# Francis-Rings/MotionEditor

Hardware: AMD Instinct MI355X
Metric: denoise-steps/sec, 24f x 512^2 two-branch UNet3D+ControlNet(+adapter+K/V injection) (higher is better)
Workload: dtype f16

## Files before the change

motioneditor_amd/csrc/gemm.hip:

```cpp
#include "me_common.h"
#include "../../include/motioned.h"
#include <stdio.h>
#include <stdlib.h>

namespace {

constexpr int BK = 64;
#ifndef WIDE_TERMS
#define WIDE_TERMS 0
#endif
constexpr int STAGE_REG = 0, STAGE_GLDS = 1, STAGE_BUF = 2;
constexpr int ROWEPI_FLAG = 1 << 30, TILEORDER_FLAG = 1 << 29;

template <bool NT = false>
__device__ __forceinline__ void st16(f16* p, uint4 v) {
  if constexpr (NT) {
    typedef unsigned u32x4 __attribute__((ext_vector_type(4)));
    __builtin_nontemporal_store((u32x4){v.x, v.y, v.z, v.w}, reinterpret_cast<u32x4*>(p));
  } else {
    *reinterpret_cast<uint4*>(p) = v;
  }
}
template <bool NT = false>
__device__ __forceinline__ void st8(f16* p, uint2 v) {
  if constexpr (NT) {
    typedef unsigned u32x2 __attribute__((ext_vector_type(2)));
    __builtin_nontemporal_store((u32x2){v.x, v.y}, reinterpret_cast<u32x2*>(p));
  } else {
    *reinterpret_cast<uint2*>(p) = v;
  }
}

__device__ uint4 g_zero16;

struct RowInfo {
  int base, y0, x0;
  bool valid;
};

__device__ __forceinline__ RowInfo make_row(const me_gemm_args& a, int m) {
  RowInfo r;
  r.valid = m < a.M;
  r.base = m;
  r.y0 = 0;
  r.x0 = 0;
  if (!r.valid) return r;
  if (a.gather == ME_GATHER_CONV3) {
    const int hw = a.Hout * a.Wout;
    const int img = m / hw;
    const int rem = m - img * hw;
    const int oy = rem / a.Wout;
    const int ox = rem - oy * a.Wout;
    r.base = img * a.Hin * a.Win;
    r.y0 = oy * a.stride - (a.pad0 ? 0 : 1);
    r.x0 = ox * a.stride - (a.pad0 ? 0 : 1);
  } else if (a.gather == ME_GATHER_TCONV) {
    const int bf = m / a.npix;
    r.y0 = bf % a.frames;
    r.x0 = (bf / a.frames) * a.npix + (m - bf * a.npix);
  }
  return r;
}

__device__ __forceinline__ int src_row(const me_gemm_args& a, const RowInfo& r, int tap) {
  if (!r.valid) return -1;
  if (a.gather == ME_GATHER_DENSE) return r.base;
  if (a.gather == ME_GATHER_CONV3) {
    const int ky = tap / 3, kx = tap - ky * 3;
    const int iy = r.y0 + ky, ix = r.x0 + kx;
    const int sh = a.ups ? 1 : 0;
    const int Hv = a.Hin << sh, Wv = a.Win << sh;
    if (iy < 0 || iy >= Hv || ix < 0 || ix >= Wv) return -1;
    if (a.ups == 2 && ((iy | ix) & 1)) return -1;
    return r.base + (iy >> sh) * a.Win + (ix >> sh);
  }
  const int dt = tap - 1;
  const int ftot = a.frames_total > 0 ? a.frames_total : a.frames;
  const int gf = a.frame0 + r.y0, gs = gf + dt;
  if (gs < 0 || gs >= ftot || gs / a.chunk != gf / a.chunk) return -1;
  const int ls = r.y0 + dt;
  if (ls >= 0 && ls < a.frames) return r.base + dt * a.npix;
  const int hb = ls < 0 ? a.halo_prev : a.halo_next;
  return hb < 0 ? -1 : hb + r.x0;
}

template <int NT, int MT, int WN>
__device__ __forceinline__ void init_acc(const me_gemm_args& a, f32x4 (&acc)[NT][MT], int n0, int wn, int lane, bool use_bias = true) {
  const f16* __restrict__ bias = use_bias ? reinterpret_cast<const f16*>(a.bias) : nullptr;
  const int nb = n0 + wn * WN + (lane >> 4) * 4;
  const float inv_alpha = bias ? 1.0f / a.alpha : 0.f;
#pragma unroll
  for (int j = 0; j < NT; ++j) {
    U64 b;
    b.u = (bias && nb + 16 * j < a.N) ? *reinterpret_cast<const uint2*>(bias + nb + 16 * j) : make_uint2(0u, 0u);
    const f32x4 v = {(float)b.e[0] * inv_alpha, (float)b.e[1] * inv_alpha, (float)b.e[2] * inv_alpha, (float)b.e[3] * inv_alpha};
#pragma unroll
    for (int i = 0; i < MT; ++i) acc[j][i] = v;
  }
}

template <int NT, int MT>
__device__ __forceinline__ void ln_fold_acc(const me_gemm_args& a, f32x4 (&acc)[NT][MT], int mbase, int nbase, int lane) {
  const float* __restrict__ st = reinterpret_cast<const float*>(a.ln_stats);
  const float* __restrict__ cs = reinterpret_cast<const float*>(a.ln_colsum);
  const float* __restrict__ cv = reinterpret_cast<const float*>(a.ln_cvec);
  const float invK = 1.0f / (float)a.K;
  float nmean[MT], rstd[MT];
#pragma unroll
  for (int i = 0; i < MT; ++i) {
    const int m = min(mbase + i * 16 + (lane & 15), a.M - 1);
    float s1 = 0.f, s2 = 0.f;
    for (int p = 0; p < a.ln_parts; ++p) {
      const f32x2 v = *reinterpret_cast<const f32x2*>(st + (long)p * a.ln_stride + 2 * (long)m);
      s1 += v[0];
      s2 += v[1];
    }
    const float mu = s1 * invK;
    const float var = __builtin_fmaf(-mu, mu, s2 * invK);
    nmean[i] = -mu;
    rstd[i] = rsqrtf(fmaxf(var, 0.f) + a.ln_eps);
  }
#pragma unroll
  for (int j = 0; j < NT; ++j) {
    const int n = nbase + j * 16 + (lane >> 4) * 4;
    f32x4 s = {0.f, 0.f, 0.f, 0.f}, c = {0.f, 0.f, 0.f, 0.f};
    if (n < a.N) {
      s = *reinterpret_cast<const f32x4*>(cs + n);
      c = *reinterpret_cast<const f32x4*>(cv + n);
    }
#pragma unroll
    for (int i = 0; i < MT; ++i)
#pragma unroll
      for (int r = 0; r < 4; ++r) acc[j][i][r] = __builtin_fmaf(rstd[i], __builtin_fmaf(nmean[i], s[r], acc[j][i][r]), c[r]);
  }
}

constexpr int LN_LDS_BYTES = 12288, LN_LDS_COLSUM = 8192, LN_LDS_CVEC = 10240;
template <int NT, int MT>
__device__ __forceinline__ void ln_fold_acc_lds(const me_gemm_args& a, f32x4 (&acc)[NT][MT], const char* img, int rloc, int cloc, int lane) {
  const float invK = 1.0f / (float)a.K;
  uint2 v[MT][4];
#pragma unroll
  for (int i = 0; i < MT; ++i) {
    const int row = rloc + i * 16 + (lane & 15);
#pragma unroll
    for (int p = 0; p < 4; ++p) v[i][p] = *reinterpret_cast<const uint2*>(img + p * 2048 + row * 8);
  }
  float nmean[MT], rstd[MT];
#pragma unroll
  for (int i = 0; i < MT; ++i) {
    float s1 = 0.f, s2 = 0.f;
#pragma unroll
    for (int p = 0; p < 4; ++p) {
      s1 += __uint_as_float(v[i][p].x);
      s2 += __uint_as_float(v[i][p].y);
    }
    const float mu = s1 * invK;
    const float var = __builtin_fmaf(-mu, mu, s2 * invK);
    nmean[i] = -mu;
    rstd[i] = rsqrtf(fmaxf(var, 0.f) + a.ln_eps);
  }
#pragma unroll
  for (int j = 0; j < NT; ++j) {
    const int col = cloc + j * 16 + (lane >> 4) * 4;
    const uint4 su = *reinterpret_cast<const uint4*>(img + LN_LDS_COLSUM + col * 4), cu = *reinterpret_cast<const uint4*>(img + LN_LDS_CVEC + col * 4);
    const f32x4 s = {__uint_as_float(su.x), __uint_as_float(su.y), __uint_as_float(su.z), __uint_as_float(su.w)};
    const f32x4 c = {__uint_as_float(cu.x), __uint_as_float(cu.y), __uint_as_float(cu.z), __uint_as_float(cu.w)};
#pragma unroll
    for (int i = 0; i < MT; ++i)
#pragma unroll
      for (int r = 0; r < 4; ++r) acc[j][i][r] = __builtin_fmaf(rstd[i], __builtin_fmaf(nmean[i], s[r], acc[j][i][r]), c[r]);
  }
}

template <int F, int NT, int MT, int WN, class RowFn>
__device__ __forceinline__ void epilogue_rows(const me_gemm_args& a, f32x4 (&acc)[NT][MT], RowFn rowfn, int m0, int n0, int wn, int lane, f16* sC, int CLD) {
  static_assert(F >= 0 && (F & 1) == 0, "specialised epilogue");
  const f16* __restrict__ rowvec = reinterpret_cast<const f16*>(a.rowvec);
  const f16* res = reinterpret_cast<const f16*>(a.res);
  const f16* res2 = reinterpret_cast<const f16*>(a.res2);
  f16* C = reinterpret_cast<f16*>(a.C);
  constexpr bool has_rv = (F & 2) != 0, has_res = (F & 4) != 0, has_res2 = (F & 8) != 0;
  const int nb = n0 + wn * WN + (lane >> 4) * 4;
  union P4 { f16x2 h[2]; uint2 u; };
  P4 o[MT][NT];
  int mrow[MT];
  auto rr = [&](int m) { return a.res_rows > 0 ? m % a.res_rows : m; };
  auto rr2 = [&](int m) { return a.res2_rows > 0 ? m % a.res2_rows : m; };
#pragma unroll
  for (int i = 0; i < MT; ++i) {
    mrow[i] = rowfn(i);
#pragma unroll
    for (int j = 0; j < NT; ++j) {
      o[i][j].h[0] = __builtin_convertvector((f32x2){acc[j][i][0] * a.alpha, acc[j][i][1] * a.alpha}, f16x2);
      o[i][j].h[1] = __builtin_convertvector((f32x2){acc[j][i][2] * a.alpha, acc[j][i][3] * a.alpha}, f16x2);
    }
  }
  const bool wide = (F == 0 || WIDE_TERMS) && sC == nullptr && a.N % 8 == 0 && a.ldc % 8 == 0 && (reinterpret_cast<uintptr_t>(a.C) & 15) == 0 &&
                    (!has_rv || (a.ldrv % 8 == 0 && (reinterpret_cast<uintptr_t>(a.rowvec) & 15) == 0)) &&
                    (!has_res || (a.ldr % 8 == 0 && (reinterpret_cast<uintptr_t>(a.res) & 15) == 0)) &&
                    (!has_res2 || (a.ldr2 % 8 == 0 && (reinterpret_cast<uintptr_t>(a.res2) & 15) == 0));
  constexpr int NP = NT / 2;
  const int gq = lane >> 4;
  if (wide) {
    union P8 { f16x2 h[4]; uint4 u; };
    const int nw = n0 + wn * WN + ((gq & 1) ? 16 + 4 * (gq - 1) : 4 * gq);
    P8 w[MT][NP > 0 ? NP : 1];
#pragma unroll
    for (int i = 0; i < MT; ++i)
#pragma unroll
      for (int jp = 0; jp < NP; ++jp) {
        const auto rx = __builtin_amdgcn_permlane16_swap(o[i][2 * jp].u.x, o[i][2 * jp + 1].u.x, false, false);
        const auto ry = __builtin_amdgcn_permlane16_swap(o[i][2 * jp].u.y, o[i][2 * jp + 1].u.y, false, false);
        w[i][jp].u = make_uint4(rx[0], ry[0], rx[1], ry[1]);
      }
    auto add_wide = [&](const f16* src, auto rowoff) {
      P8 t[MT][NP > 0 ? NP : 1];
#pragma unroll
      for (int i = 0; i < MT; ++i) {
        const f16* p = src + rowoff(mrow[i] < 0 ? 0 : mrow[i]) + nw;
#pragma unroll
        for (int jp = 0; jp < NP; ++jp) t[i][jp].u = nw + 32 * jp + 7 < a.N ? *reinterpret_cast<const uint4*>(p + 32 * jp) : make_uint4(0u, 0u, 0u, 0u);
      }
#pragma unroll
      for (int i = 0; i < MT; ++i)
#pragma unroll
        for (int jp = 0; jp < NP; ++jp)
#pragma unroll
          for (int q = 0; q < 4; ++q) w[i][jp].h[q] += t[i][jp].h[q];
    };
    auto add_narrow_last = [&](const f16* src, auto rowoff) {
      if constexpr (NT % 2 == 1) {
#pragma unroll
        for (int i = 0; i < MT; ++i) {
          P4 t;
          t.u = nb + 16 * (NT - 1) < a.N ? *reinterpret_cast<const uint2*>(src + rowoff(mrow[i] < 0 ? 0 : mrow[i]) + nb + 16 * (NT - 1)) : make_uint2(0u, 0u);
          o[i][NT - 1].h[0] += t.h[0];
          o[i][NT - 1].h[1] += t.h[1];
        }
      }
    };
    if constexpr (has_rv) { add_wide(rowvec, [&](int m) { return (long)(m / a.rows_per_vec) * a.ldrv; }); add_narrow_last(rowvec, [&](int m) { return (long)(m / a.rows_per_vec) * a.ldrv; }); }
    if constexpr (has_res) { add_wide(res, [&](int m) { return (long)rr(m) * a.ldr; }); add_narrow_last(res, [&](int m) { return (long)rr(m) * a.ldr; }); }
    if constexpr (has_res2) { add_wide(res2, [&](int m) { return (long)rr2(m) * a.ldr2; }); add_narrow_last(res2, [&](int m) { return (long)rr2(m) * a.ldr2; }); }
    if constexpr (F == 0) {
      if (a.C2) {
        f16* C2 = reinterpret_cast<f16*>(a.C2);
        long hoff[NP + 1];
#pragma unroll
        for (int jp = 0; jp <= NP; ++jp) {
          const int col = jp < NP ? nw + 32 * jp : nb + 16 * (NT - 1);
          const int n2 = col - a.c2_col0, hh = n2 / a.c2_dh;
          hoff[jp] = n2 >= 0 ? (long)hh * a.c2_hs + (n2 - hh * a.c2_dh) : -1;
        }
#pragma unroll
        for (int i = 0; i < MT; ++i) {
          if (mrow[i] < 0) continue;
          f16* crow = C + (long)mrow[i] * a.ldc;
          f16* hrow = C2 + (long)mrow[i] * a.c2_dh;
#pragma unroll
          for (int jp = 0; jp < NP; ++jp)
            if (nw + 32 * jp + 7 < a.N) st16(hoff[jp] >= 0 ? hrow + hoff[jp] : crow + nw + 32 * jp, w[i][jp].u);
          if constexpr (NT % 2 == 1) {
            if (nb + 16 * (NT - 1) < a.N) st8(hoff[NP] >= 0 ? hrow + hoff[NP] : crow + nb + 16 * (NT - 1), o[i][NT - 1].u);
          }
        }
        return;
      }
    }
#pragma unroll
    for (int i = 0; i < MT; ++i) {
      if (mrow[i] < 0) continue;
      f16* crow = C + (long)mrow[i] * a.ldc;
#pragma unroll
      for (int jp = 0; jp < NP; ++jp)
        if (nw + 32 * jp + 7 < a.N) st16(crow + nw + 32 * jp, w[i][jp].u);
      if constexpr (NT % 2 == 1) {
        if (nb + 16 * (NT - 1) < a.N) st8(crow + nb + 16 * (NT - 1), o[i][NT - 1].u);
      }
    }
    return;
  }
  auto add_term = [&](const f16* src, auto rowoff) {
    P4 t[MT][NT];
#pragma unroll
    for (int i = 0; i < MT; ++i) {
      const f16* p = src + rowoff(mrow[i] < 0 ? 0 : mrow[i]) + nb;
#pragma unroll
      for (int j = 0; j < NT; ++j) t[i][j].u = nb + 16 * j < a.N ? *reinterpret_cast<const uint2*>(p + 16 * j) : make_uint2(0u, 0u);
    }
#pragma unroll
    for (int i = 0; i < MT; ++i)
#pragma unroll
      for (int j = 0; j < NT; ++j) {
        o[i][j].h[0] += t[i][j].h[0];
        o[i][j].h[1] += t[i][j].h[1];
      }
  };
  if constexpr (has_rv) add_term(rowvec, [&](int m) { return (long)(m / a.rows_per_vec) * a.ldrv; });
  if constexpr (has_res) add_term(res, [&](int m) { return (long)rr(m) * a.ldr; });
  if constexpr (has_res2) add_term(res2, [&](int m) { return (long)rr2(m) * a.ldr2; });
  if constexpr (F == 0) {
    if (a.C2 && sC == nullptr) {
      f16* C2 = reinterpret_cast<f16*>(a.C2);
#pragma unroll
      for (int j = 0; j < NT; ++j) {
        const int col = nb + 16 * j;
        if (col >= a.N) continue;
        const int n2 = col - a.c2_col0, hh = n2 / a.c2_dh;
        const long hoff = n2 >= 0 ? (long)hh * a.c2_hs + (n2 - hh * a.c2_dh) : -1;
#pragma unroll
        for (int i = 0; i < MT; ++i) {
          if (mrow[i] < 0) continue;
          st8(hoff >= 0 ? C2 + (long)mrow[i] * a.c2_dh + hoff : C + (long)mrow[i] * a.ldc + col, o[i][j].u);
        }
      }
      return;
    }
  }
#pragma unroll
  for (int i = 0; i < MT; ++i) {
    if (mrow[i] < 0) continue;
    f16* crow = C + (long)mrow[i] * a.ldc + nb;
    f16* lrow = sC + (mrow[i] - m0) * CLD + (nb - n0);
#pragma unroll
    for (int j = 0; j < NT; ++j) {
      if (nb + 16 * j >= a.N) continue;
      if (sC) *reinterpret_cast<uint2*>(lrow + 16 * j) = o[i][j].u;
      else st8(crow + 16 * j, o[i][j].u);
    }
  }
}

struct LnOutCtx { int m0, wr, wc, tid; char* red; };
template <int F, int NT, int MT, int WN>
__device__ __forceinline__ void epilogue_rowpass(const me_gemm_args& a, f32x4 (&acc)[NT][MT], int mw0, int nw0, int lane, char* scr, const LnOutCtx& lnx) {
  static_assert(F >= 0 && (F & 1) == 0 && MT % 2 == 0 && WN % 16 == 0, "row-pass epilogue");
  constexpr bool has_rv = (F & 2) != 0, has_res = (F & 4) != 0, has_res2 = (F & 8) != 0;
  constexpr int NCHK = MT / 2, ROWS = 32, CH = WN / 8, PIECES = ROWS * CH, IT = PIECES / 64, PITCH = WN * 2 + 16;
  static_assert(PIECES % 64 == 0, "whole instructions per chunk");
  const f16* __restrict__ rowvec = reinterpret_cast<const f16*>(a.rowvec);
  const f16* res = reinterpret_cast<const f16*>(a.res);
  const f16* res2 = reinterpret_cast<const f16*>(a.res2);
  f16* C = reinterpret_cast<f16*>(a.C);
  union P4 { f16x2 h[2]; uint2 u; };
  union P8 { f16x2 h[4]; uint4 u; };
  P4 o[MT][NT];
#pragma unroll
  for (int i = 0; i < MT; ++i)
#pragma unroll
    for (int j = 0; j < NT; ++j) {
      o[i][j].h[0] = __builtin_convertvector((f32x2){acc[j][i][0] * a.alpha, acc[j][i][1] * a.alpha}, f16x2);
      o[i][j].h[1] = __builtin_convertvector((f32x2){acc[j][i][2] * a.alpha, acc[j][i][3] * a.alpha}, f16x2);
    }
  int prow[IT], pcol[IT], poff[IT];
#pragma unroll
  for (int t = 0; t < IT; ++t) {
    const int p = t * 64 + lane;
    prow[t] = p / CH;
    pcol[t] = nw0 + (p - prow[t] * CH) * 8;
    poff[t] = prow[t] * PITCH + (p - prow[t] * CH) * 16;
  }
  constexpr int TH = MT * 16;
  const int mwc = min(mw0, a.M - 1);
  int v0 = 0, vb = 0x7fffffff, r0 = 0, q0 = 0;
  if constexpr (has_rv) { v0 = mwc / a.rows_per_vec; vb = (v0 + 1) * a.rows_per_vec; }
  if constexpr (has_res) r0 = a.res_rows > 0 ? mwc % a.res_rows : 0;
  if constexpr (has_res2) q0 = a.res2_rows > 0 ? mwc % a.res2_rows : 0;
  auto vrow = [&](int m) { return a.rows_per_vec >= TH ? v0 + (m >= vb ? 1 : 0) : m / a.rows_per_vec; };
  auto wrap = [&](int m, int period, int first) {
    if (period <= 0) return m;
    if (period < TH) return m % period;
    const int x = first + (m - mwc);
    return x >= period ? x - period : x;
  };
  constexpr int NRES = (has_res ? 1 : 0) + (has_res2 ? 1 : 0), NRV = NRES > 0 ? NRES : 1;
  bool rv_once = false;
  P8 rvp[has_rv ? IT : 1];
  if constexpr (has_rv) {
    const int mlast = max(min(mw0 + TH, a.M) - 1, mwc);
    rv_once = vrow(mwc) == vrow(mlast);
    if (rv_once) {
#pragma unroll
      for (int t = 0; t < IT; ++t) rvp[t].u = *reinterpret_cast<const uint4*>(rowvec + (long)vrow(mwc) * a.ldrv + pcol[t]);
    }
  }
  auto load_rv = [&](int c) {
#pragma unroll
    for (int t = 0; t < IT; ++t) {
      const int m = min(mw0 + c * ROWS + prow[t], a.M - 1);
      rvp[t].u = *reinterpret_cast<const uint4*>(rowvec + (long)vrow(m) * a.ldrv + pcol[t]);
    }
  };
  auto load_terms = [&](int c, P8 (&tv)[NRV][IT]) {
#pragma unroll
    for (int t = 0; t < IT; ++t) {
      const int m = min(mw0 + c * ROWS + prow[t], a.M - 1);
      int k = 0;
      if constexpr (has_res) tv[k++][t].u = *reinterpret_cast<const uint4*>(res + (long)wrap(m, a.res_rows, r0) * a.ldr + pcol[t]);
      if constexpr (has_res2) tv[k++][t].u = *reinterpret_cast<const uint4*>(res2 + (long)wrap(m, a.res2_rows, q0) * a.ldr2 + pcol[t]);
    }
  };
  const int wrow = lane & 15, wq = lane >> 4;
  auto park = [&](int c, P8 (&d)[IT]) {
#pragma unroll
    for (int ii = 0; ii < 2; ++ii)
#pragma unroll
      for (int j = 0; j < NT; ++j) *reinterpret_cast<uint2*>(scr + (ii * 16 + wrow) * PITCH + (j * 16 + wq * 4) * 2) = o[c * 2 + ii][j].u;
#pragma unroll
    for (int t = 0; t < IT; ++t) d[t].u = *reinterpret_cast<const uint4*>(scr + poff[t]);
  };
  auto add_rv = [&](P8 (&d)[IT]) {
#pragma unroll
    for (int t = 0; t < IT; ++t)
#pragma unroll
      for (int q = 0; q < 4; ++q) d[t].h[q] += rvp[t].h[q];
  };
  auto add_terms = [&](P8 (&d)[IT], P8 (&tv)[NRV][IT]) {
#pragma unroll
    for (int k = 0; k < NRES; ++k)
#pragma unroll
      for (int t = 0; t < IT; ++t)
#pragma unroll
        for (int q = 0; q < 4; ++q) d[t].h[q] += tv[k][t].h[q];
  };
  long hoff[IT];
  const bool c2 = F == 0 && a.C2 != nullptr;
  if (c2) {
#pragma unroll
    for (int t = 0; t < IT; ++t) {
      const int n2 = pcol[t] - a.c2_col0, hh = n2 / a.c2_dh;
      hoff[t] = n2 >= 0 ? (long)hh * a.c2_hs + (n2 - hh * a.c2_dh) : -1;
    }
  }
  auto store = [&](int c, P8 (&d)[IT]) {
#pragma unroll
    for (int t = 0; t < IT; ++t) {
      const int m = mw0 + c * ROWS + prow[t];
      if (m >= a.M) continue;
      f16* dst = C + (long)m * a.ldc + pcol[t];
      if (c2 && hoff[t] >= 0) dst = reinterpret_cast<f16*>(a.C2) + (long)m * a.c2_dh + hoff[t];
      st16(dst, d[t].u);
    }
  };
  const bool lnout = a.ln_out != nullptr;
  static_assert(CH % 2 == 0, "row sums: half the pieces of a row per half wave");
  f32x2 rsum[NCHK];
  auto row_sums = [&](int c, P8 (&d)[IT]) {
    const f16x2 one2 = {(f16)1.f, (f16)1.f};
#pragma unroll
    for (int t = 0; t < IT; ++t) {
      float s1 = 0.f, s2 = 0.f;
#pragma unroll
      for (int q = 0; q < 4; ++q) {
        s1 = __builtin_amdgcn_fdot2(d[t].h[q], one2, s1, false);
        s2 = __builtin_amdgcn_fdot2(d[t].h[q], d[t].h[q], s2, false);
      }
      const int p = t * 64 + lane;
      *reinterpret_cast<uint2*>(scr + p * 8) = make_uint2(__float_as_uint(s1), __float_as_uint(s2));
    }
    f32x2 acc2 = {0.f, 0.f};
#pragma unroll
    for (int k = 0; k < CH / 2; ++k) {
      const uint2 v = *reinterpret_cast<const uint2*>(scr + ((lane & 31) * CH + (lane >> 5) * (CH / 2) + k) * 8);
      acc2 += f32x2{__uint_as_float(v.x), __uint_as_float(v.y)};
    }
    rsum[c] = f32x2{xor32_sum(acc2[0]), xor32_sum(acc2[1])};
  };
  P8 tv[2][NRV][IT];
  if constexpr (NRES > 0) load_terms(0, tv[0]);
#pragma unroll
  for (int c = 0; c < NCHK; ++c) {
    P8 d[IT];
    if constexpr (has_rv) {
      if (!rv_once) load_rv(c);
    }
    park(c, d);
    if constexpr (has_rv) add_rv(d);
    if constexpr (NRES > 0) {
      add_terms(d, tv[c & 1]);
      if (c + 1 < NCHK) load_terms(c + 1, tv[(c + 1) & 1]);
    }
    store(c, d);
    if (lnout) row_sums(c, d);
  }
  if (lnout) {
    constexpr int GR = MT * 16;
    uint2* red = reinterpret_cast<uint2*>(lnx.red);
    if (lane < 32) {
#pragma unroll
      for (int c = 0; c < NCHK; ++c) red[(lnx.wr * 4 + lnx.wc) * GR + c * 32 + lane] = make_uint2(__float_as_uint(rsum[c][0]), __float_as_uint(rsum[c][1]));
    }
    __syncthreads();
    if (lnx.tid < 2 * GR) {
      const int g = lnx.tid / GR, r = lnx.tid - g * GR, m = lnx.m0 + lnx.tid;
      f32x2 sum = {0.f, 0.f};
#pragma unroll
      for (int w4 = 0; w4 < 4; ++w4) {
        const uint2 v = red[(g * 4 + w4) * GR + r];
        sum += f32x2{__uint_as_float(v.x), __uint_as_float(v.y)};
      }
      if (m < a.M) *reinterpret_cast<f32x2*>(reinterpret_cast<float*>(a.ln_out) + (long)((nw0 - lnx.wc * WN) / 320) * a.ln_out_stride + 2 * (long)m) = sum;
    }
  }
}

template <int NT, int MT, int WN>
__device__ __forceinline__ void epilogue_geglu_rowpass(const me_gemm_args& a, f32x4 (&acc)[NT][MT], int m0, int n0, int wr, int wc, int lane, char* tile) {
  static_assert(NT == 4 && WN == 64, "256-wide GEGLU tile: 4 waves x 32 output columns");
  constexpr int NO = NT / 2, GR = MT * 16;
  f16* C = reinterpret_cast<f16*>(a.C);
  const int wrow = lane & 15, wq = lane >> 4;
#pragma unroll
  for (int i = 0; i < MT; ++i)
#pragma unroll
    for (int jj = 0; jj < NO; ++jj) {
      float v[4];
      {
        const f32x2 v01 = geglu2(f32x2{acc[2 * jj][i][0], acc[2 * jj][i][1]}, f32x2{acc[2 * jj + 1][i][0], acc[2 * jj + 1][i][1]});
        const f32x2 v23 = geglu2(f32x2{acc[2 * jj][i][2], acc[2 * jj][i][3]}, f32x2{acc[2 * jj + 1][i][2], acc[2 * jj + 1][i][3]});
        v[0] = v01[0]; v[1] = v01[1]; v[2] = v23[0]; v[3] = v23[1];
      }
      union { f16x2 h[2]; uint2 u; } o;
      o.h[0] = __builtin_convertvector((f32x2){v[0], v[1]}, f16x2);
      o.h[1] = __builtin_convertvector((f32x2){v[2], v[3]}, f16x2);
      const int row = wr * GR + i * 16 + wrow;
      const int col = wc * 32 + jj * 16 + wq * 4;
      const int pos = (col >> 3) ^ (row & 15);
      *reinterpret_cast<uint2*>(tile + row * 256 + pos * 16 + (col & 4) * 2) = o.u;
    }
  __syncthreads();
  const int wave = wr * 4 + wc;
  constexpr int RW = 2 * GR / 8;
  const int Nout0 = n0 / 2;
#pragma unroll
  for (int t = 0; t < RW / 4; ++t) {
    const int p = t * 64 + lane, row = wave * RW + (p >> 4), pos = p & 15;
    const uint4 v = *reinterpret_cast<const uint4*>(tile + row * 256 + pos * 16);
    const int m = m0 + row, n = Nout0 + ((pos ^ (row & 15)) << 3);
    if (m < a.M) st16<true>(C + (long)m * a.ldc + n, v);
  }
}


template <int NT, int MT, int WN, class RowFn>
__device__ __forceinline__ void epilogue_generic(const me_gemm_args& a, f32x4 (&acc)[NT][MT], RowFn rowfn, int m0, int n0, int wn, int lane, f16* sC, int CLD) {
  const f16* __restrict__ rowvec = reinterpret_cast<const f16*>(a.rowvec);
  const f16* res = reinterpret_cast<const f16*>(a.res);
  const f16* res2 = reinterpret_cast<const f16*>(a.res2);
  f16* C = reinterpret_cast<f16*>(a.C);
  const int nq = (lane >> 4) * 4;
#pragma unroll
  for (int i = 0; i < MT; ++i) {
    const int m = rowfn(i);
    if (m < 0) continue;
    const f16* rv = rowvec ? rowvec + (long)(m / a.rows_per_vec) * a.ldrv : nullptr;
#pragma unroll
    for (int j = 0; j < NT; ++j) {
      const int n = n0 + wn * WN + j * 16 + nq;
      if (n >= a.N) continue;
      float v[4];
#pragma unroll
      for (int r = 0; r < 4; ++r) v[r] = acc[j][i][r] * a.alpha;
      if (rv) {
        U64 b;
        b.u = *reinterpret_cast<const uint2*>(rv + n);
#pragma unroll
        for (int r = 0; r < 4; ++r) v[r] += (float)b.e[r];
      }
      if (a.act == 1) {
#pragma unroll
        for (int r = 0; r < 4; ++r) v[r] = fmaxf(v[r], 0.f);
      } else if (a.act == 2) {
#pragma unroll
        for (int r = 0; r < 4; ++r) v[r] = silu_f(v[r]);
      }
      const int mr = a.res_rows > 0 ? m % a.res_rows : m;
      if (res) {
        U64 b;
        b.u = *reinterpret_cast<const uint2*>(res + (long)mr * a.ldr + n);
#pragma unroll
        for (int r = 0; r < 4; ++r) v[r] += (float)b.e[r];
      }
      if (res2) {
        U64 b;
        b.u = *reinterpret_cast<const uint2*>(res2 + (long)(a.res2_rows > 0 ? m % a.res2_rows : m) * a.ldr2 + n);
#pragma unroll
        for (int r = 0; r < 4; ++r) v[r] += (float)b.e[r];
      }
      U64 o;
#pragma unroll
      for (int r = 0; r < 4; ++r) o.e[r] = (f16)v[r];
      if (sC) *reinterpret_cast<uint2*>(sC + (m - m0) * CLD + (n - n0)) = o.u;
      else *reinterpret_cast<uint2*>(C + (long)m * a.ldc + n) = o.u;
    }
  }
}

template <int NT, int MT, int WN, class RowFn>
__device__ __forceinline__ void epilogue_geglu(const me_gemm_args& a, f32x4 (&acc)[NT][MT], RowFn rowfn, int m0, int n0, int wn, int lane, f16* sC, int CLD) {
  f16* C = reinterpret_cast<f16*>(a.C);
  constexpr int NO = NT / 2;
  const int nb = n0 + wn * WN + (lane >> 4) * 4;
  const int nob = (n0 + wn * WN) / 2 + (lane >> 4) * 4;
  const int Nout = a.N / 2;
  union P4 { f16x2 h[2]; uint2 u; };
  P4 o[MT][NO];
  int mrow[MT];
#pragma unroll
  for (int i = 0; i < MT; ++i) {
    mrow[i] = rowfn(i);
#pragma unroll
    for (int jj = 0; jj < NO; ++jj) {
      float v[4];
      {
        const f32x2 v01 = geglu2(f32x2{acc[2 * jj][i][0], acc[2 * jj][i][1]}, f32x2{acc[2 * jj + 1][i][0], acc[2 * jj + 1][i][1]});
        const f32x2 v23 = geglu2(f32x2{acc[2 * jj][i][2], acc[2 * jj][i][3]}, f32x2{acc[2 * jj + 1][i][2], acc[2 * jj + 1][i][3]});
        v[0] = v01[0]; v[1] = v01[1]; v[2] = v23[0]; v[3] = v23[1];
      }
      o[i][jj].h[0] = __builtin_convertvector((f32x2){v[0], v[1]}, f16x2);
      o[i][jj].h[1] = __builtin_convertvector((f32x2){v[2], v[3]}, f16x2);
    }
  }
  const bool wide = sC == nullptr && Nout % 8 == 0 && a.ldc % 8 == 0 && (reinterpret_cast<uintptr_t>(a.C) & 15) == 0;
  constexpr int NP = NO / 2;
  const int gq = lane >> 4;
  const int nw = (n0 + wn * WN) / 2 + ((gq & 1) ? 16 + 4 * (gq - 1) : 4 * gq);
#pragma unroll
  for (int i = 0; i < MT; ++i) {
    const int m = mrow[i];
    if (wide) {
#pragma unroll
      for (int jp = 0; jp < NP; ++jp) {
        const auto rx = __builtin_amdgcn_permlane16_swap(o[i][2 * jp].u.x, o[i][2 * jp + 1].u.x, false, false);
        const auto ry = __builtin_amdgcn_permlane16_swap(o[i][2 * jp].u.y, o[i][2 * jp + 1].u.y, false, false);
        if (m >= 0 && nw + 32 * jp + 7 < Nout) st16<true>(C + (long)m * a.ldc + nw + 32 * jp, make_uint4(rx[0], ry[0], rx[1], ry[1]));
      }
      if constexpr (NO % 2 == 1) {
        if (m >= 0 && nob + 16 * (NO - 1) < Nout) st8<true>(C + (long)m * a.ldc + nob + 16 * (NO - 1), o[i][NO - 1].u);
      }
      continue;
    }
    if (m < 0) continue;
#pragma unroll
    for (int jj = 0; jj < NO; ++jj) {
      if (nb + 32 * jj >= a.N) continue;
      const int no = nob + 16 * jj;
      if (sC) *reinterpret_cast<uint2*>(sC + (m - m0) * CLD + (no - n0 / 2)) = o[i][jj].u;
      else st8<true>(C + (long)m * a.ldc + no, o[i][jj].u);
    }
  }
}

template <int NT, int MT, int WN, class RowFn>
__device__ __forceinline__ void epilogue(const me_gemm_args& a, f32x4 (&acc)[NT][MT], RowFn rowfn, int m0, int n0, int wn, int lane, f16* sC, int CLD) {
  if (a.geglu) return epilogue_geglu<NT, MT, WN>(a, acc, rowfn, m0, n0, wn, lane, sC, CLD);
  const int f = a.act != 0 ? -1 : ((a.rowvec ? 2 : 0) | (a.res ? 4 : 0) | (a.res2 ? 8 : 0));
  switch (f) {
    case 0: return epilogue_rows<0, NT, MT, WN>(a, acc, rowfn, m0, n0, wn, lane, sC, CLD);
    case 2: return epilogue_rows<2, NT, MT, WN>(a, acc, rowfn, m0, n0, wn, lane, sC, CLD);
    case 4: return epilogue_rows<4, NT, MT, WN>(a, acc, rowfn, m0, n0, wn, lane, sC, CLD);
    case 6: return epilogue_rows<6, NT, MT, WN>(a, acc, rowfn, m0, n0, wn, lane, sC, CLD);
    case 12: return epilogue_rows<12, NT, MT, WN>(a, acc, rowfn, m0, n0, wn, lane, sC, CLD);
    default: return epilogue_generic<NT, MT, WN>(a, acc, rowfn, m0, n0, wn, lane, sC, CLD);
  }
}

template <int BM, int BN, int STAGE, int WM = 64>
__global__ __launch_bounds__(BM / WM * 128, WM == 128 ? 1 : 2) void gemm_kernel(const me_gemm_args a) {
  constexpr int NTHR = BM / WM * 128;
  constexpr int RSTR = NTHR / 8;
  constexpr int WN = BN / 2;
  constexpr int NT = WN / 16;
  constexpr int MT = WM / 16;
  constexpr int XROWS = BM / RSTR;
  constexpr int WROWS = BN / RSTR;
  constexpr int LD = STAGE != STAGE_REG ? BK : BK + 8;

  extern __shared__ __attribute__((aligned(16))) char smem[];
  f16* sX = reinterpret_cast<f16*>(smem);
  f16* sW = sX + 2 * BM * LD;

  const int tid = threadIdx.x;
  const int lane = tid & 63;
  const int wave = __builtin_amdgcn_readfirstlane(tid >> 6);
  const int wm = wave >> 1, wn = wave & 1;

  const int nbn = (a.N + BN - 1) / BN;
  const int nbm = (a.M - a.m_off + BM - 1) / BM;
  const int w = xcd_remap(blockIdx.x, nbm * nbn);
  const int tile_n = w % nbn, tile_m = w / nbn;
  const int m0 = a.m_off + tile_m * BM, n0 = tile_n * BN;

  const f16* __restrict__ X = reinterpret_cast<const f16*>(a.X);
  const f16* __restrict__ W = reinterpret_cast<const f16*>(a.W);

  const int taps = a.gather == ME_GATHER_CONV3 ? 9 : (a.gather == ME_GATHER_TCONV ? 3 : 1);
  const int nkc = (a.K + BK - 1) / BK;
  const bool packk = STAGE == STAGE_GLDS && a.gather == ME_GATHER_CONV3 && a.K < BK && BK % a.K == 0;
  const int nit = packk ? (9 * a.K + BK - 1) / BK : taps * nkc;

  int srow, scol;
  if (STAGE != STAGE_REG) {
    srow = wave * 8 + (lane >> 3);
    scol = ((lane & 7) ^ ((4 * (wave & 1) + (lane >> 4)) & 7)) * 8;
  } else {
    srow = tid >> 3;
    scol = (tid & 7) * 8;
  }

  RowInfo rinfo[XROWS];
#pragma unroll
  for (int i = 0; i < XROWS; ++i) rinfo[i] = make_row(a, m0 + srow + RSTR * i);

  long xoff[XROWS];
  int cur_tap = -1;
  auto set_tap = [&](int tap) {
    if (tap != cur_tap) {
      cur_tap = tap;
#pragma unroll
      for (int i = 0; i < XROWS; ++i) {
        const int s = src_row(a, rinfo[i], tap);
        xoff[i] = s < 0 ? -1L : (long)s * a.ldx;
      }
    }
  };

  const int S = STAGE == STAGE_BUF ? a.splits_ : 0;
  const int it0 = S > 1 ? (int)((long)nit * blockIdx.y / S) : 0;
  const int it1 = S > 1 ? (int)((long)nit * (blockIdx.y + 1) / S) : nit;
  f32x4 acc[NT][MT];
  init_acc<NT, MT, WN>(a, acc, n0, wn, lane, S <= 1);

  const int frow = lane & 15;
  const int fg = lane >> 4;

  auto compute = [&](int buf) {
    const f16* bx = sX + buf * BM * LD;
    const f16* bw = sW + buf * BN * LD;
#pragma unroll
    for (int ks = 0; ks < BK / 32; ++ks) {
      f16x8 fx[MT], fw[NT];
#pragma unroll
      for (int i = 0; i < MT; ++i) {
        const int row = wm * WM + i * 16 + frow;
        const int ch = STAGE != STAGE_REG ? ((ks * 4 + fg) ^ ((row >> 1) & 7)) : (ks * 4 + fg);
        fx[i] = *reinterpret_cast<const f16x8*>(bx + row * LD + ch * 8);
      }
#pragma unroll
      for (int j = 0; j < NT; ++j) {
        const int row = wn * WN + j * 16 + frow;
        const int ch = STAGE != STAGE_REG ? ((ks * 4 + fg) ^ ((row >> 1) & 7)) : (ks * 4 + fg);
        fw[j] = *reinterpret_cast<const f16x8*>(bw + row * LD + ch * 8);
      }
#pragma unroll
      for (int j = 0; j < NT; ++j)
#pragma unroll
        for (int i = 0; i < MT; ++i) acc[j][i] = mfma16(fw[j], fx[i], acc[j][i]);
    }
  };

  if constexpr (STAGE == STAGE_BUF) {
    typedef __attribute__((address_space(3))) void* lptr_t;
    constexpr unsigned OOB = 0x80000000u;
    long brow = m0;
    if (a.gather == ME_GATHER_CONV3) brow = (long)(m0 / (a.Hout * a.Wout)) * a.Hin * a.Win;
    else if (a.gather == ME_GATHER_TCONV) brow = m0 > a.npix ? m0 - a.npix : 0;
    const auto xsrd = __builtin_amdgcn_make_buffer_rsrc(const_cast<f16*>(X + brow * a.ldx), 0, OOB, 0x00020000);
    const int wrows = min(a.N - n0, BN);
    const auto wsrd = __builtin_amdgcn_make_buffer_rsrc(const_cast<f16*>(W + (long)n0 * taps * a.K), 0, (unsigned)((long)wrows * taps * a.K * 2), 0x00020000);
    unsigned xo[XROWS], wo[WROWS];
#pragma unroll
    for (int i = 0; i < WROWS; ++i) wo[i] = (unsigned)(((long)(srow + RSTR * i) * taps * a.K + scol) * 2);
    auto set_tap_off = [&](int tap) {
#pragma unroll
      for (int i = 0; i < XROWS; ++i) {
        const int sr = src_row(a, rinfo[i], tap);
        xo[i] = sr < 0 ? OOB : (unsigned)(((long)(sr - brow) * a.ldx + scol) * 2);
      }
    };
    int tap_l = it0 / nkc, kc_l = it0 - (it0 / nkc) * nkc;
    set_tap_off(tap_l);
    auto gload = [&](int buf) {
      char* dx = reinterpret_cast<char*>(sX + buf * BM * LD) + wave * 1024;
      char* dw = reinterpret_cast<char*>(sW + buf * BN * LD) + wave * 1024;
      const int sx = kc_l * (BK * 2), sw = (tap_l * a.K + kc_l * BK) * 2;
#pragma unroll
      for (int i = 0; i < XROWS; ++i) __builtin_amdgcn_raw_ptr_buffer_load_lds(xsrd, (lptr_t)(dx + i * (RSTR * 128)), 16, (int)xo[i], sx, 0, 0);
#pragma unroll
      for (int i = 0; i < WROWS; ++i) __builtin_amdgcn_raw_ptr_buffer_load_lds(wsrd, (lptr_t)(dw + i * (RSTR * 128)), 16, (int)wo[i], sw, 0, 0);
      if (++kc_l == nkc) {
        kc_l = 0;
        if (++tap_l < taps) set_tap_off(tap_l);
      }
    };
    gload(0);
    __syncthreads();
    for (int it = it0; it < it1; ++it) {
      const int buf = (it - it0) & 1;
      if (it + 1 < it1) gload(buf ^ 1);
      compute(buf);
      __syncthreads();
    }
    if (S > 1) {
      float* wk = reinterpret_cast<float*>(a.work) + (long)blockIdx.y * a.M * a.N;
#pragma unroll
      for (int i = 0; i < MT; ++i) {
        const int m = m0 + wm * WM + i * 16 + (lane & 15);
        if (m >= a.M) continue;
#pragma unroll
        for (int j = 0; j < NT; ++j) {
          const int n = n0 + wn * WN + j * 16 + (lane >> 4) * 4;
          if (n < a.N) *reinterpret_cast<f32x4*>(wk + (long)m * a.N + n) = acc[j][i];
        }
      }
      return;
    }
  } else if constexpr (STAGE == STAGE_GLDS) {
    typedef const __attribute__((address_space(1))) void* gptr_t;
    typedef __attribute__((address_space(3))) void* lptr_t;
    const f16* zsrc = reinterpret_cast<const f16*>(&g_zero16);
    auto gload = [&](int it, int buf) {
      int tap = it / nkc;
      int c = (it - tap * nkc) * BK + scol;
      bool kok = c < a.K;
      long wk = (long)tap * a.K + c;
      if (packk) {
        wk = it * BK + scol;
        tap = (int)wk / a.K;
        c = (int)wk - tap * a.K;
        kok = tap < 9;
        if (!kok) tap = 8;
      }
      set_tap(tap);
      char* dx = reinterpret_cast<char*>(sX + buf * BM * LD) + wave * 1024;
      char* dw = reinterpret_cast<char*>(sW + buf * BN * LD) + wave * 1024;
#pragma unroll
      for (int i = 0; i < XROWS; ++i) {
        const f16* src = (kok && xoff[i] >= 0) ? X + xoff[i] + c : zsrc;
        __builtin_amdgcn_global_load_lds((gptr_t)src, (lptr_t)(dx + i * (RSTR * 128)), 16, 0, 0);
      }
#pragma unroll
      for (int i = 0; i < WROWS; ++i) {
        const int n = n0 + srow + RSTR * i;
        const f16* src = (kok && n < a.N) ? W + (long)n * taps * a.K + wk : zsrc;
        __builtin_amdgcn_global_load_lds((gptr_t)src, (lptr_t)(dw + i * (RSTR * 128)), 16, 0, 0);
      }
    };
    gload(0, 0);
    __syncthreads();
    for (int it = 0; it < nit; ++it) {
      const int buf = it & 1;
      if (it + 1 < nit) gload(it + 1, buf ^ 1);
      compute(buf);
      __syncthreads();
    }
  } else {
    uint4 rx[XROWS], rw[WROWS];
    auto gload = [&](int it) {
      const int tap = it / nkc;
      const int c = (it - tap * nkc) * BK + scol;
      set_tap(tap);
      const bool kok = c < a.K;
#pragma unroll
      for (int i = 0; i < XROWS; ++i) rx[i] = (kok && xoff[i] >= 0) ? ldg128(X + xoff[i] + c) : zero128();
#pragma unroll
      for (int i = 0; i < WROWS; ++i) {
        const int n = n0 + srow + RSTR * i;
        rw[i] = (kok && n < a.N) ? ldg128(W + ((long)n * taps + tap) * a.K + c) : zero128();
      }
    };
    auto sstore = [&](int buf) {
      f16* dx = sX + buf * BM * LD;
      f16* dw = sW + buf * BN * LD;
#pragma unroll
      for (int i = 0; i < XROWS; ++i) *reinterpret_cast<uint4*>(dx + (srow + RSTR * i) * LD + scol) = rx[i];
#pragma unroll
      for (int i = 0; i < WROWS; ++i) *reinterpret_cast<uint4*>(dw + (srow + RSTR * i) * LD + scol) = rw[i];
    };
    gload(0);
    sstore(0);
    __syncthreads();
    for (int it = 0; it < nit; ++it) {
      const int buf = it & 1;
      if (it + 1 < nit) gload(it + 1);
      compute(buf);
      if (it + 1 < nit) sstore(buf ^ 1);
      __syncthreads();
    }
  }

  if (a.ln_stats) ln_fold_acc<NT, MT>(a, acc, m0 + wm * WM, n0 + wn * WN, lane);
  const int ncols = a.geglu ? BN / 2 : BN;
  const int Nout = a.geglu ? a.N / 2 : a.N;
  constexpr bool CFITS = (size_t)BM * (BN + 8) <= (size_t)2 * (BM + BN) * LD;
  const bool wide_store = CFITS && (Nout % 8 == 0) && (a.ldc % 8 == 0) && ((reinterpret_cast<uintptr_t>(a.C) & 15) == 0) && !a.C2;
  auto rowfn = [&](int i) {
    const int m = m0 + wm * WM + i * 16 + (lane & 15);
    return m < a.M ? m : -1;
  };
  if (!wide_store) {
    epilogue<NT, MT, WN>(a, acc, rowfn, m0, n0, wn, lane, nullptr, 0);
    return;
  }
  constexpr int CLD = BN + 8;
  f16* sC = reinterpret_cast<f16*>(smem);
  epilogue<NT, MT, WN>(a, acc, rowfn, m0, n0, wn, lane, sC, CLD);
  __syncthreads();
  f16* C = reinterpret_cast<f16*>(a.C);
  const int vpr = ncols / 8;
  const int nb0 = a.geglu ? n0 / 2 : n0;
  for (int idx = tid; idx < BM * vpr; idx += NTHR) {
    const int row = idx / vpr, c8 = (idx - row * vpr) * 8;
    const int m = m0 + row, n = nb0 + c8;
    if (m < a.M && n < Nout) *reinterpret_cast<uint4*>(C + (long)m * a.ldc + n) = *reinterpret_cast<const uint4*>(sC + row * CLD + c8);
  }
}

constexpr int HALO_W = 18, HALO_ROWS = HALO_W * HALO_W, HALO_INSTR = (HALO_ROWS + 7) / 8;
constexpr int HALO_BYTES = HALO_INSTR * 1024, CONVW_BYTES = 320 * 128;

__global__ __launch_bounds__(512, 2) void conv3_halo_kernel(const me_gemm_args a) {
  constexpr int BN = 320, WN = 160, NT = 10, MT = 4;
  extern __shared__ __attribute__((aligned(16))) char smem[];
  char* sH = smem;
  char* sWt = smem + HALO_BYTES;

  const int tid = threadIdx.x;
  const int lane = tid & 63;
  const int wave = __builtin_amdgcn_readfirstlane(tid >> 6);
  const int wm = wave >> 1, wn = wave & 1;

  const int nbn = a.N / BN;
  const int tx_n = a.Win >> 4, ppi = tx_n * (a.Hin >> 4);
  const int hw = a.Hin * a.Win;
  const int w = xcd_remap(blockIdx.x, (a.M / hw) * ppi * nbn);
  const int tile_n = w % nbn, patch = w / nbn;
  const int img = patch / ppi, pr = patch - img * ppi;
  const int ty = pr / tx_n, tx = pr - ty * tx_n;
  const int y0 = ty * 16, x0 = tx * 16, n0 = tile_n * BN;

  const f16* __restrict__ X = reinterpret_cast<const f16*>(a.X);
  const f16* __restrict__ W = reinterpret_cast<const f16*>(a.W);

  const int srow = wave * 8 + (lane >> 3);
  const int scol = ((lane & 7) ^ ((4 * (wave & 1) + (lane >> 4)) & 7)) * 8;
  typedef __attribute__((address_space(3))) void* lptr_t;
  constexpr unsigned OOB = 0x80000000u;
  const auto xsrd = __builtin_amdgcn_make_buffer_rsrc(const_cast<f16*>(X + (long)img * hw * a.ldx), 0, OOB, 0x00020000);
  const auto wsrd = __builtin_amdgcn_make_buffer_rsrc(const_cast<f16*>(W + (long)n0 * 9 * a.K), 0, (unsigned)((long)BN * 9 * a.K * 2), 0x00020000);
  unsigned hoff[6];
#pragma unroll
  for (int i = 0; i < 6; ++i) {
    const int hr = srow + 64 * i;
    unsigned o = OOB;
    if (hr < HALO_ROWS) {
      const int hy = hr / HALO_W, hx = hr - hy * HALO_W;
      const int iy = y0 - 1 + hy, ix = x0 - 1 + hx;
      if (iy >= 0 && iy < a.Hin && ix >= 0 && ix < a.Win) o = (unsigned)(((long)(iy * a.Win + ix) * a.ldx + scol) * 2);
    }
    hoff[i] = o;
  }
  auto load_halo = [&](int kc) {
#pragma unroll
    for (int i = 0; i < 6; ++i) {
      if (wave + 8 * i < HALO_INSTR)
        __builtin_amdgcn_raw_ptr_buffer_load_lds(xsrd, (lptr_t)(sH + (wave + 8 * i) * 1024), 16, (int)hoff[i], kc * (BK * 2), 0, 0);
    }
  };
  unsigned woff[5];
#pragma unroll
  for (int i = 0; i < 5; ++i) woff[i] = (unsigned)(((long)(srow + 64 * i) * 9 * a.K + scol) * 2);
  auto load_w = [&](int tap, int kc, int buf) {
    char* dw = sWt + buf * CONVW_BYTES + wave * 1024;
    const int so = (tap * a.K + kc * BK) * 2;
#pragma unroll
    for (int i = 0; i < 5; ++i) __builtin_amdgcn_raw_ptr_buffer_load_lds(wsrd, (lptr_t)(dw + i * 8192), 16, (int)woff[i], so, 0, 0);
  };

  f32x4 acc[NT][MT];
  init_acc<NT, MT, WN>(a, acc, n0, wn, lane);

  const int frow = lane & 15, fg = lane >> 4;
  auto compute = [&](int tap, int buf) {
    const int ky = tap / 3, kx = tap - ky * 3;
    const char* bw = sWt + buf * CONVW_BYTES;
    const int hbase = (wm * 4 + ky) * HALO_W + kx + frow;
#pragma unroll
    for (int ks = 0; ks < BK / 32; ++ks) {
      f16x8 fx[MT], fw[NT];
#pragma unroll
      for (int i = 0; i < MT; ++i) {
        const int row = hbase + i * HALO_W;
        fx[i] = *reinterpret_cast<const f16x8*>(sH + row * 128 + (((ks * 4 + fg) ^ ((row >> 1) & 7)) << 4));
      }
#pragma unroll
      for (int j = 0; j < NT; ++j) {
        const int row = wn * WN + j * 16 + frow;
        fw[j] = *reinterpret_cast<const f16x8*>(bw + row * 128 + (((ks * 4 + fg) ^ ((row >> 1) & 7)) << 4));
      }
#pragma unroll
      for (int j = 0; j < NT; ++j)
#pragma unroll
        for (int i = 0; i < MT; ++i) acc[j][i] = mfma16(fw[j], fx[i], acc[j][i]);
    }
  };

  const int nkc = a.K / BK;
  load_halo(0);
  load_w(0, 0, 0);
  __syncthreads();
  int it = 0;
  for (int kc = 0; kc < nkc; ++kc) {
    for (int tap = 0; tap < 9; ++tap, ++it) {
      const int buf = it & 1;
      const bool last_tap = tap == 8;
      if (!last_tap) load_w(tap + 1, kc, buf ^ 1);
      else if (kc + 1 < nkc) load_w(0, kc + 1, buf ^ 1);
      compute(tap, buf);
      if (last_tap && kc + 1 < nkc) {
        __syncthreads();
        load_halo(kc + 1);
      }
      __syncthreads();
    }
  }

  auto rowfn = [&](int i) { return img * hw + (y0 + wm * 4 + i) * a.Win + x0 + (lane & 15); };
  epilogue<NT, MT, WN>(a, acc, rowfn, 0, n0, wn, lane, nullptr, 0);
}

template <int BM, int BN, bool GATHER, int EPI>
__global__ __launch_bounds__(512, 2) void gemm8p_kernel(const me_gemm_args a) {
  constexpr int WN = BN / 4, NT = WN / 16, NT0 = (NT + 1) / 2, NT1 = NT / 2;
  constexpr int GR = BM / 2, HALF = GR / 2, MH = HALF / 16, MT = 2 * MH;
  constexpr int NPA = 2 * HALF / 8;
  constexpr int ABYTES = BM * 128, BUFBYTES = (BM + BN) * 128;
  static_assert(BN % 64 == 0 && NT1 >= 1 && HALF % 16 == 0 && NPA >= 8 && NPA <= 16, "wave tile");
  extern __shared__ __attribute__((aligned(16))) char smem[];

  const int tid = threadIdx.x;
  const int lane = tid & 63;
  const int wave = __builtin_amdgcn_readfirstlane(tid >> 6);
  const int wr = wave >> 2, wc = wave & 3;

  const int nbn = (a.N + BN - 1) / BN;
  const int nbm = (a.M - a.m_off + BM - 1) / BM;
  const int w = xcd_remap(blockIdx.x, nbm * nbn);
  int tile_n, tile_m;
  if (a.splits_ & TILEORDER_FLAG) { tile_m = w % nbm; tile_n = w / nbm; }
  else { tile_n = w % nbn; tile_m = w / nbn; }
  const int m0 = a.m_off + tile_m * BM, n0 = tile_n * BN;

  const f16* __restrict__ X = reinterpret_cast<const f16*>(a.X);
  const f16* __restrict__ W = reinterpret_cast<const f16*>(a.W);
  const int taps = !GATHER ? 1 : (a.gather == ME_GATHER_CONV3 ? 9 : (a.gather == ME_GATHER_TCONV ? 3 : 1));
  const int nkc = a.K / BK;
  const int nit = taps * nkc;

  typedef __attribute__((address_space(3))) void* lptr_t;
  constexpr unsigned OOB = 0x80000000u;
  long brow = m0;
  if (GATHER) {
    if (a.gather == ME_GATHER_CONV3) brow = (long)(m0 / (a.Hout * a.Wout)) * a.Hin * a.Win;
    else if (a.gather == ME_GATHER_TCONV) brow = m0 > a.npix ? m0 - a.npix : 0;
  }
  const auto xsrd = __builtin_amdgcn_make_buffer_rsrc(const_cast<f16*>(X + brow * a.ldx), 0, OOB, 0x00020000);
  const int wrows = min(a.N - n0, BN);
  const auto wsrd = __builtin_amdgcn_make_buffer_rsrc(const_cast<f16*>(W + (long)n0 * taps * a.K), 0, (unsigned)((long)wrows * taps * a.K * 2), 0x00020000);

  const int prow = lane >> 3;
  const int scol = ((lane & 7) ^ ((4 * (wave & 1) + (lane >> 4)) & 7)) * 8;
  int rA[2][2], rB0[NT0], rB1[NT1];
#pragma unroll
  for (int i = 0; i < 2; ++i) {
    const int p = wave + 8 * i;
    rA[0][i] = __builtin_amdgcn_readfirstlane((p / (HALF / 8)) * GR + 8 * (p % (HALF / 8)));
    rA[1][i] = __builtin_amdgcn_readfirstlane((p / (HALF / 8)) * GR + HALF + 8 * (p % (HALF / 8)));
  }
  const bool two_a = __builtin_amdgcn_readfirstlane(wave + 8 < NPA ? 1 : 0) != 0;
#pragma unroll
  for (int i = 0; i < NT0; ++i) {
    const int p = wave + 8 * i;
    rB0[i] = __builtin_amdgcn_readfirstlane((p / (2 * NT0)) * WN + 8 * (p % (2 * NT0)));
  }
#pragma unroll
  for (int i = 0; i < NT1; ++i) {
    const int p = wave + 8 * i;
    rB1[i] = __builtin_amdgcn_readfirstlane((p / (2 * NT1)) * WN + 16 * NT0 + 8 * (p % (2 * NT1)));
  }

  unsigned* tab = reinterpret_cast<unsigned*>(smem + 2 * BUFBYTES);
  unsigned xo[2][2];
  if constexpr (GATHER) {
    const int r = tid & 255;
    const RowInfo ri = make_row(a, r < BM ? m0 + r : a.M);
    for (int tap = tid >> 8; tap < taps; tap += 2) {
      const int sr = src_row(a, ri, tap);
      tab[tap * 256 + r] = sr < 0 ? OOB : (unsigned)((long)(sr - brow) * a.ldx * 2);
    }
    __syncthreads();
  } else {
#pragma unroll
    for (int h = 0; h < 2; ++h)
#pragma unroll
      for (int i = 0; i < 2; ++i) {
        const int m = m0 + rA[h][i] + prow;
        xo[h][i] = (m < a.M && (i == 0 || two_a)) ? (unsigned)(((long)(m - brow) * a.ldx + scol) * 2) : OOB;
      }
  }
  unsigned wo0[NT0], wo1[NT1];
#pragma unroll
  for (int i = 0; i < NT0; ++i) wo0[i] = (unsigned)(((long)(rB0[i] + prow) * taps * a.K + scol) * 2);
#pragma unroll
  for (int i = 0; i < NT1; ++i) wo1[i] = (unsigned)(((long)(rB1[i] + prow) * taps * a.K + scol) * 2);

  struct Cur { int tap, kc, tl; };
  Cur cA0 = {0, 0, 0}, cA1 = {0, 0, 0};
  int tB0 = 0, tB1 = 0;
  auto issueA = [&](Cur& c, int half) {
    char* base = smem + (c.tl & 1) * BUFBYTES;
    const int sx = __builtin_amdgcn_readfirstlane((GATHER ? c.kc : c.tl) * (BK * 2));
    const bool live = c.tl < nit;
    unsigned v[2];
#pragma unroll
    for (int i = 0; i < 2; ++i) {
      if constexpr (GATHER) v[i] = tab[__builtin_amdgcn_readfirstlane(min(c.tap, taps - 1)) * 256 + min(rA[half][i] + prow, 255)] + (unsigned)(scol * 2);
      else v[i] = xo[half][i];
    }
    __builtin_amdgcn_raw_ptr_buffer_load_lds(xsrd, (lptr_t)(base + rA[half][0] * 128), 16, (int)(live ? v[0] : OOB), sx, 0, 0);
    if (BM == 256 || two_a) __builtin_amdgcn_raw_ptr_buffer_load_lds(xsrd, (lptr_t)(base + rA[half][1] * 128), 16, (int)(live ? v[1] : OOB), sx, 0, 0);
    ++c.tl;
    if constexpr (GATHER) {
      if (++c.kc == nkc) { c.kc = 0; ++c.tap; }
    }
  };
  auto issueB0 = [&]() {
    char* base = smem + (tB0 & 1) * BUFBYTES + ABYTES;
    const int sw = __builtin_amdgcn_readfirstlane(tB0 * (BK * 2));
    const bool live = tB0 < nit;
#pragma unroll
    for (int i = 0; i < NT0; ++i)
      __builtin_amdgcn_raw_ptr_buffer_load_lds(wsrd, (lptr_t)(base + rB0[i] * 128), 16, (int)(live ? wo0[i] : OOB), sw, 0, 0);
    ++tB0;
  };
  auto issueB1 = [&]() {
    char* base = smem + (tB1 & 1) * BUFBYTES + ABYTES;
    const int sw = __builtin_amdgcn_readfirstlane(tB1 * (BK * 2));
    const bool live = tB1 < nit;
#pragma unroll
    for (int i = 0; i < NT1; ++i)
      __builtin_amdgcn_raw_ptr_buffer_load_lds(wsrd, (lptr_t)(base + rB1[i] * 128), 16, (int)(live ? wo1[i] : OOB), sw, 0, 0);
    ++tB1;
  };

  f32x4 acc[NT][MT];
  init_acc<NT, MT, WN>(a, acc, n0, wc, lane);

  const int frow = lane & 15, fg = lane >> 4;
  const int c0 = (fg ^ ((frow >> 1) & 7)) << 4;
  const int la0 = (wr * GR + frow) * 128 + c0, la1 = la0 ^ 64;
  const int lb0 = ABYTES + (wc * WN + frow) * 128 + c0, lb1 = lb0 ^ 64;
  f16x8 fa[2][MH], fb[2][NT0];
  auto readA = [&](int buf, int half) {
#pragma unroll
    for (int i = 0; i < MH; ++i) {
      fa[0][i] = *reinterpret_cast<const f16x8*>(smem + buf * BUFBYTES + la0 + (half * MH + i) * 2048);
      fa[1][i] = *reinterpret_cast<const f16x8*>(smem + buf * BUFBYTES + la1 + (half * MH + i) * 2048);
    }
  };
  auto readB = [&](int buf, int j0, int nj) {
#pragma unroll
    for (int j = 0; j < NT0; ++j) {
      if (j < nj) {
        fb[0][j] = *reinterpret_cast<const f16x8*>(smem + buf * BUFBYTES + lb0 + (j0 + j) * 2048);
        fb[1][j] = *reinterpret_cast<const f16x8*>(smem + buf * BUFBYTES + lb1 + (j0 + j) * 2048);
      }
    }
  };
  auto cluster = [&](int half, int j0, int nj) {
    __builtin_amdgcn_s_setprio(1);
#pragma unroll
    for (int ks = 0; ks < 2; ++ks)
#pragma unroll
      for (int j = 0; j < NT0; ++j)
        if (j < nj) {
#pragma unroll
          for (int i = 0; i < MH; ++i) acc[j0 + j][half * MH + i] = mfma16(fb[ks][j], fa[ks][i], acc[j0 + j][half * MH + i]);
        }
    __builtin_amdgcn_s_setprio(0);
  };
#define ME_BAR()                               \
  do {                                         \
    __builtin_amdgcn_sched_barrier(0);         \
    asm volatile("" ::: "memory");             \
    __builtin_amdgcn_s_barrier();              \
    asm volatile("" ::: "memory");             \
    __builtin_amdgcn_sched_barrier(0);         \
  } while (0)
#define ME_LGKM0()                                       \
  do {                                                   \
    asm volatile("s_waitcnt lgkmcnt(0)" ::: "memory");   \
    __builtin_amdgcn_sched_barrier(0);                   \
  } while (0)

  auto wait_young = [&]() {
    static_assert(NT1 == 2, "vmcnt literals below");
    if (BM == 256 || two_a) asm volatile("s_waitcnt vmcnt(4)" ::: "memory");
    else asm volatile("s_waitcnt vmcnt(3)" ::: "memory");
  };
  constexpr bool LN_LDS = EPI == 0 && !GATHER;
  if constexpr (LN_LDS) {
    if (a.ln_stats) {
      constexpr int np = 8;
      for (int q = wave; q < np + 4; q += 8) {
        const char* src;
        unsigned range;
        int dst;
        if (q < np) {
          const bool live = (q >> 1) < a.ln_parts;
          src = reinterpret_cast<const char*>(a.ln_stats) + (live ? ((long)(q >> 1) * a.ln_stride + 2 * (long)m0) * 4 : 0L);
          range = live ? (unsigned)min(a.M - m0, BM) * 8u : 0u;
          dst = (q >> 1) * 2048 + (q & 1) * 1024;
        } else {
          const int k = q - np;
          src = reinterpret_cast<const char*>((k >> 1) ? a.ln_cvec : a.ln_colsum) + (long)n0 * 4;
          range = (unsigned)min(a.N - n0, BN) * 4u;
          dst = ((k >> 1) ? LN_LDS_CVEC : LN_LDS_COLSUM) + (k & 1) * 1024;
        }
        const auto srd = __builtin_amdgcn_make_buffer_rsrc(const_cast<char*>(src), 0, range, 0x00020000);
        __builtin_amdgcn_raw_ptr_buffer_load_lds(srd, (lptr_t)(smem + 2 * BUFBYTES + dst), 16, (q & 1) * 1024 + lane * 16, 0, 0, 0);
      }
    }
  }
  issueA(cA0, 0);
  issueB0();
  issueB1();
  issueA(cA1, 1);
  issueA(cA0, 0);
  issueB1();
  wait_young();
  ME_BAR();
  if (wr == 1) ME_BAR();

  for (int t = 0; t < nit; ++t) {
    const int buf = t & 1;
    readB(buf, 0, NT0);
    readA(buf, 0);
    issueA(cA1, 1);
    ME_BAR();
    ME_LGKM0();
    cluster(0, 0, NT0);
    ME_BAR();
    readB(buf, NT0, NT1);
    issueB0();
    ME_BAR();
    ME_LGKM0();
    cluster(0, NT0, NT1);
    ME_BAR();
    readA(buf, 1);
    issueA(cA0, 0);
    ME_BAR();
    ME_LGKM0();
    cluster(1, NT0, NT1);
    ME_BAR();
    readB(buf, 0, NT0);
    issueB1();
    wait_young();
    ME_BAR();
    ME_LGKM0();
    cluster(1, 0, NT0);
    ME_BAR();
  }
  if (wr == 0) ME_BAR();
  asm volatile("s_waitcnt vmcnt(0)" ::: "memory");
#undef ME_BAR
#undef ME_LGKM0

  if constexpr (EPI <= 0) {
    if (a.ln_stats) {
      if constexpr (LN_LDS) ln_fold_acc_lds<NT, MT>(a, acc, smem + 2 * BUFBYTES, wr * GR, wc * WN, lane);
      else ln_fold_acc<NT, MT>(a, acc, m0 + wr * GR, n0 + wc * WN, lane);
    }
  }

  if constexpr (EPI >= 0 && BN == 256) {
    __builtin_amdgcn_s_barrier();
    return epilogue_geglu_rowpass<NT, MT, WN>(a, acc, m0, n0, wr, wc, lane, smem);
  } else if constexpr (EPI >= 0) {
    __builtin_amdgcn_s_barrier();
    char* scr = smem + wave * (32 * (WN * 2 + 16));
    const int mw0 = m0 + wr * GR, nw0 = n0 + wc * WN;
    const LnOutCtx lnx = {m0, wr, wc, tid, smem + 8 * (32 * (WN * 2 + 16))};
    return epilogue_rowpass<EPI, NT, MT, WN>(a, acc, mw0, nw0, lane, scr, lnx);
  } else {
    auto rowfn = [&](int i) {
      const int m = m0 + wr * GR + i * 16 + (lane & 15);
      return m < a.M ? m : -1;
    };
    epilogue<NT, MT, WN>(a, acc, rowfn, m0, n0, wc, lane, nullptr, 0);
  }
}

__global__ __launch_bounds__(256) void gemm_splitk_reduce_kernel(const me_gemm_args a) {
  const int vpr = a.N / 4;
  const long total = (long)a.M * vpr;
  const float* __restrict__ wk = reinterpret_cast<const float*>(a.work);
  const f16* __restrict__ bias = reinterpret_cast<const f16*>(a.bias);
  const f16* __restrict__ rowvec = reinterpret_cast<const f16*>(a.rowvec);
  const f16* res = reinterpret_cast<const f16*>(a.res);
  const f16* res2 = reinterpret_cast<const f16*>(a.res2);
  f16* C = reinterpret_cast<f16*>(a.C);
  const long plane = (long)a.M * a.N;
  for (long idx = (long)blockIdx.x * 256 + threadIdx.x; idx < total; idx += (long)gridDim.x * 256) {
    const int m = (int)(idx / vpr);
    const int n = (int)(idx - (long)m * vpr) * 4;
    f32x4 v = *reinterpret_cast<const f32x4*>(wk + (long)m * a.N + n);
    for (int s_ = 1; s_ < a.splits_; ++s_) v += *reinterpret_cast<const f32x4*>(wk + s_ * plane + (long)m * a.N + n);
    v *= a.alpha;
    if (bias) {
      U64 b;
      b.u = *reinterpret_cast<const uint2*>(bias + n);
#pragma unroll
      for (int r = 0; r < 4; ++r) v[r] += (float)b.e[r];
    }
    U64 rv, r1, r2, o;
    if (rowvec) rv.u = *reinterpret_cast<const uint2*>(rowvec + (long)(m / a.rows_per_vec) * a.ldrv + n);
    if (res) r1.u = *reinterpret_cast<const uint2*>(res + (long)(a.res_rows > 0 ? m % a.res_rows : m) * a.ldr + n);
    if (res2) r2.u = *reinterpret_cast<const uint2*>(res2 + (long)(a.res2_rows > 0 ? m % a.res2_rows : m) * a.ldr2 + n);
    if (a.act == 0) {
#pragma unroll
      for (int r = 0; r < 4; ++r) {
        f16 h = (f16)v[r];
        if (rowvec) h = h + rv.e[r];
        if (res) h = h + r1.e[r];
        if (res2) h = h + r2.e[r];
        o.e[r] = h;
      }
    } else {
#pragma unroll
      for (int r = 0; r < 4; ++r) {
        float f = v[r];
        if (rowvec) f += (float)rv.e[r];
        f = a.act == 1 ? fmaxf(f, 0.f) : silu_f(f);
        if (res) f += (float)r1.e[r];
        if (res2) f += (float)r2.e[r];
        o.e[r] = (f16)f;
      }
    }
    *reinterpret_cast<uint2*>(C + (long)m * a.ldc + n) = o.u;
  }
}

long split_below() {
  const char* e = getenv("ME_GEMM_SPLITK");
  return e ? atol(e) : 400;
}
int choose_split(const me_gemm_args* a, long blocks, int nit) {
  if (a->geglu || a->K % 64 || a->N < 1280 || blocks >= split_below() || nit < 32 || a->C2 || a->m_off || a->ln_stats) return 1;
  int S = (int)((640 + blocks - 1) / blocks);
  if (S > 4) S = 4;
  if (S > nit / 4) S = nit / 4;
  return S < 2 ? 1 : S;
}

int stage_impl() {
  static int impl = -1;
  if (impl < 0) {
    const char* e = getenv("ME_GEMM_STAGE");
    impl = (e && e[0] == 'r') ? STAGE_REG : STAGE_GLDS;
  }
  return impl;
}

long big_min_blocks() {
  static long v = -1;
  if (v < 0) {
    const char* e = getenv("ME_GEMM_BIG_MIN");
    v = e ? atol(e) : 512;
  }
  return v;
}

long halo_min_blocks() {
  static long v = -1;
  if (v < 0) {
    const char* e = getenv("ME_CONV_HALO_MIN");
    v = e ? atol(e) : 512;
  }
  return v;
}

bool conv_halo() {
  static int on = -1;
  if (on < 0) {
    const char* e = getenv("ME_CONV_HALO");
    on = (e && e[0] == '0') ? 0 : 1;
  }
  return on == 1;
}

bool buf_stage() {
  static int on = -1;
  if (on < 0) {
    const char* e = getenv("ME_GEMM_BUF");
    on = (e && e[0] == '0') ? 0 : 1;
  }
  return on == 1;
}

int use_8p() {
  const char* e = getenv("ME_GEMM_8P");
  return e ? atoi(e) : 2;
}

bool row_epilogue() {
  const char* e = getenv("ME_GEMM_ROWEPI");
  return !(e && e[0] == '0');
}

bool tile_order_exp() {
  static int on = -1;
  if (on < 0) {
    const char* e = getenv("ME_GEMM_TILE_ORDER");
    on = (e && e[0] == '1') ? 1 : 0;
  }
  return on == 1;
}

long min_tiles_192() {
  const char* e = getenv("ME_GEMM_8P_192");
  const long v = e ? atol(e) : 192;
  return v > 0 ? v : (1L << 60);
}

long min_tiles_128() {
  const char* e = getenv("ME_GEMM_8P_128");
  const long v = e ? atol(e) : 192;
  return v > 0 ? v : (1L << 60);
}

long geglu_min_tiles() {
  const char* e = getenv("ME_GEMM_GEGLU_MIN");
  return e ? atol(e) : 240;
}

int min_ktiles_192() {
  const char* e = getenv("ME_GEMM_192_MINK");
  return e ? atoi(e) : 4;
}

long n64_below() {
  const char* e = getenv("ME_GEMM_N64_BELOW");
  return e ? atol(e) : 200;
}

bool tile160() {
  static int on = -1;
  if (on < 0) {
    const char* e = getenv("ME_GEMM_TILE160");
    on = (e && e[0] == '0') ? 0 : 1;
  }
  return on == 1;
}

}

extern "C" void me_set_error(const char* msg);
extern "C" void me_set_kernel(const char* name);
extern "C" const char* me_last_kernel(void);

static thread_local bool g_ln_fused = false;

template <int BM, int BN, int STAGE, int WM = 64>
static int launch_gemm(const me_gemm_args* a, hipStream_t st) {
  const size_t lds = (size_t)2 * (BM + BN) * (STAGE != STAGE_REG ? BK : BK + 8) * sizeof(f16);
  static bool attr_set_dev[64] = {};
  int dev_id = 0;
  (void)hipGetDevice(&dev_id);
  bool& attr_set = attr_set_dev[dev_id & 63];
  if (!attr_set) {
    if (hipFuncSetAttribute(reinterpret_cast<const void*>(&gemm_kernel<BM, BN, STAGE, WM>), hipFuncAttributeMaxDynamicSharedMemorySize, (int)lds) != hipSuccess) {
      me_set_error("me_gemm: hipFuncSetAttribute(MaxDynamicSharedMemorySize) failed");
      return ME_EHIP;
    }
    attr_set = true;
  }
  const int nbm = (a->M - a->m_off + BM - 1) / BM, nbn = (a->N + BN - 1) / BN;
  (void)hipGetLastError();
  me_gemm_args b = *a;
  b.splits_ = 0;
  int S = 1;
  if (STAGE == STAGE_BUF && a->work) {
    const int nit = (a->K / 64) * (a->gather == ME_GATHER_CONV3 ? 9 : (a->gather == ME_GATHER_TCONV ? 3 : 1));
    const int Msel = a->sel_rows > a->M ? a->sel_rows : a->M;
    S = choose_split(a, (long)((Msel + BM - 1) / BM) * nbn, nit);
    if ((int64_t)S * a->M * a->N * 4 > a->work_bytes || a->N % 4 || ((uintptr_t)a->work & 15)) S = 1;
  }
  if (S > 1) {
    b.splits_ = S;
    hipLaunchKernelGGL((gemm_kernel<BM, BN, STAGE, WM>), dim3(nbm * nbn, S), dim3(BM / WM * 128), lds, st, b);
    const long vec = (long)a->M * (a->N / 4);
    hipLaunchKernelGGL(gemm_splitk_reduce_kernel, dim3((unsigned)((vec + 255) / 256 < 4096 ? (vec + 255) / 256 : 4096)), dim3(256), 0, st, b);
  } else {
    hipLaunchKernelGGL((gemm_kernel<BM, BN, STAGE, WM>), dim3(nbm * nbn), dim3(BM / WM * 128), lds, st, b);
  }
  {
    char nm[64];
    snprintf(nm, sizeof(nm), "gemm_kernel<%d,%d%s>%s", BM, BN, STAGE == STAGE_REG ? ",reg" : "", S > 1 ? "+splitk" : "");
    me_set_kernel(nm);
  }
  if (hipGetLastError() != hipSuccess) {
    me_set_error("me_gemm: kernel launch failed");
    return ME_EHIP;
  }
  return ME_OK;
}

template <int BM, int BN, bool GATHER, int EPI>
static int launch_gemm8p_epi(const me_gemm_args& b, hipStream_t st) {
  const int lds = 2 * (BM + BN) * 128 + (GATHER ? 9 * 256 * 4 : (EPI == 0 ? LN_LDS_BYTES : 0));
  static bool attr_set_dev[64] = {};
  int dev_id = 0;
  (void)hipGetDevice(&dev_id);
  bool& attr_set = attr_set_dev[dev_id & 63];
  if (!attr_set) {
    if (hipFuncSetAttribute(reinterpret_cast<const void*>(&gemm8p_kernel<BM, BN, GATHER, EPI>), hipFuncAttributeMaxDynamicSharedMemorySize, lds) != hipSuccess) {
      me_set_error("me_gemm: hipFuncSetAttribute(MaxDynamicSharedMemorySize) failed");
      return ME_EHIP;
    }
    attr_set = true;
  }
  const int nbm = (b.M - b.m_off + BM - 1) / BM, nbn = (b.N + BN - 1) / BN;
  hipLaunchKernelGGL((gemm8p_kernel<BM, BN, GATHER, EPI>), dim3(nbm * nbn), dim3(512), lds, st, b);
  return ME_OK;
}

template <int BM, int BN, bool GATHER>
static int launch_gemm8p(const me_gemm_args* a, hipStream_t st) {
  (void)hipGetLastError();
  me_gemm_args b = *a;
  b.splits_ = 0;
  int epi = -1;
  {
    auto al = [](const void* p, int ld) { return p == nullptr || (ld % 8 == 0 && (reinterpret_cast<uintptr_t>(p) & 15) == 0); };
    const int f = (a->rowvec ? 2 : 0) | (a->res ? 4 : 0) | (a->res2 ? 8 : 0);
    if (BN == 320 && row_epilogue() && !a->geglu && a->act == 0 && a->N % 320 == 0 && (f == 0 || f == 2 || f == 4 || f == 6 || f == 12) && al(a->C, a->ldc) &&
        al(a->rowvec, a->ldrv) && al(a->res, a->ldr) && al(a->res2, a->ldr2) && (!a->C2 || f == 0))
      epi = f;
    if (tile_order_exp()) b.splits_ |= TILEORDER_FLAG;
    if (BN == 256 && BM == 256 && row_epilogue() && a->geglu && a->N % 256 == 0 && al(a->C, a->ldc) && !a->C2) epi = 0;
    if (epi >= 0) b.splits_ |= ROWEPI_FLAG;
    g_ln_fused = BN == 320 && epi >= 0 && a->ln_out != nullptr;
    if (!g_ln_fused) b.ln_out = nullptr;
  }
  int rc;
  if constexpr (BN == 256) {
    rc = epi == 0 ? launch_gemm8p_epi<BM, BN, GATHER, 0>(b, st) : launch_gemm8p_epi<BM, BN, GATHER, -1>(b, st);
  } else {
    switch (epi) {
      case 0: rc = launch_gemm8p_epi<BM, BN, GATHER, 0>(b, st); break;
      case 2: rc = launch_gemm8p_epi<BM, BN, GATHER, 2>(b, st); break;
      case 4: rc = launch_gemm8p_epi<BM, BN, GATHER, 4>(b, st); break;
      case 6: rc = launch_gemm8p_epi<BM, BN, GATHER, 6>(b, st); break;
      case 12: rc = launch_gemm8p_epi<BM, BN, GATHER, 12>(b, st); break;
      default: rc = launch_gemm8p_epi<BM, BN, GATHER, -1>(b, st); break;
    }
  }
  if (rc != ME_OK) return rc;
  {
    char nm[64];
    snprintf(nm, sizeof(nm), "gemm8p_kernel<%d,%d,%s>", BM, BN, GATHER ? "true" : "false");
    me_set_kernel(nm);
  }
  if (hipGetLastError() != hipSuccess) {
    me_set_error("me_gemm: kernel launch failed");
    return ME_EHIP;
  }
  return ME_OK;
}

static int launch_conv_halo(const me_gemm_args* a, hipStream_t st) {
  const int lds = HALO_BYTES + 2 * CONVW_BYTES;
  static bool attr_set_dev[64] = {};
  int dev_id = 0;
  (void)hipGetDevice(&dev_id);
  bool& attr_set = attr_set_dev[dev_id & 63];
  if (!attr_set) {
    if (hipFuncSetAttribute(reinterpret_cast<const void*>(&conv3_halo_kernel), hipFuncAttributeMaxDynamicSharedMemorySize, lds) != hipSuccess) {
      me_set_error("me_gemm: hipFuncSetAttribute(MaxDynamicSharedMemorySize) failed");
      return ME_EHIP;
    }
    attr_set = true;
  }
  const long blocks = (long)(a->M / 256) * (a->N / 320);
  (void)hipGetLastError();
  hipLaunchKernelGGL(conv3_halo_kernel, dim3((unsigned)blocks), dim3(512), lds, st, *a);
  me_set_kernel("conv3_halo_kernel");
  if (hipGetLastError() != hipSuccess) {
    me_set_error("me_gemm: kernel launch failed");
    return ME_EHIP;
  }
  return ME_OK;
}

extern "C" int64_t me_gemm_work_bytes(const me_gemm_args* a) {
  if (!a || a->M <= 0 || a->N <= 0 || a->K <= 0 || a->geglu || a->K % 64 || a->N % 4) return 0;
  const int nit = (a->K / 64) * (a->gather == ME_GATHER_CONV3 ? 9 : (a->gather == ME_GATHER_TCONV ? 3 : 1));
  const long blocks = (long)((a->M + 127) / 128) * ((a->N + 159) / 160);
  const int S = choose_split(a, blocks, nit);
  return S > 1 ? (int64_t)4 * a->M * a->N * 4 : 0;
}

static int gemm_dispatch(const me_gemm_args* a, void* stream);

extern "C" int me_gemm(const me_gemm_args* a, void* stream) {
  if (!a || !a->X || !a->W || !a->C) { me_set_error("me_gemm: null pointer"); return ME_EINVAL; }
  if (a->ln_stats) {
    if (a->gather != ME_GATHER_DENSE || a->bias || a->alpha != 1.0f || a->rowvec || a->res || a->res2 || a->act || !a->ln_colsum || !a->ln_cvec || a->ln_parts < 1 || a->ln_parts > 4 || a->ln_stride < 2 * (int64_t)a->M ||
        (a->ln_stride & 1) || ((uintptr_t)a->ln_stats & 7) || (((uintptr_t)a->ln_colsum | (uintptr_t)a->ln_cvec) & 15) || !(a->ln_eps > 0.f)) {
      me_set_error("me_gemm: a LayerNorm-folded launch is dense, has no bias (it is inside ln_cvec), no rowvec / residual / activation and alpha == 1; ln_colsum / ln_cvec fp32 [N] 16-byte aligned, "
                   "ln_stats 8-byte aligned with 1 <= ln_parts <= 4 parts ln_stride >= 2 M floats apart, ln_eps > 0");
      return ME_EINVAL;
    }
  }
  if (a->ln_out && (a->geglu || a->C2 || a->N % 8 || a->N > 1536 || a->ldc % 8 || ((uintptr_t)a->C & 15) || ((uintptr_t)a->ln_out & 7) || a->ln_out_stride < 2 * (int64_t)a->M || (a->ln_out_stride & 1))) {
    me_set_error("me_gemm: ln_out needs a plain fp16 output of N % 8 == 0, N <= 1536 columns (no GEGLU, no head-major panels), ldc % 8 == 0, and parts >= 2 M floats apart");
    return ME_EINVAL;
  }
  g_ln_fused = false;
  const int rc = gemm_dispatch(a, stream);
  if (rc != ME_OK || !a->ln_out || g_ln_fused) return rc;
  char nm[96];
  snprintf(nm, sizeof(nm), "%s", me_last_kernel());
  const int rc2 = me_ln_stats(reinterpret_cast<const f16*>(a->C) + (long)a->m_off * a->ldc, a->ldc, (int64_t)a->M - a->m_off, a->N,
                              reinterpret_cast<float*>(a->ln_out) + 2 * (long)a->m_off, a->ln_out_stride, stream);
  me_set_kernel(nm);
  return rc2;
}

static int gemm_dispatch(const me_gemm_args* a, void* stream) {
  if (a->M <= 0 || a->N <= 0 || a->K <= 0) { me_set_error("me_gemm: non-positive dimension"); return ME_EINVAL; }
  if (a->K % 8 || a->ldx % 8 || a->ldc % 4 || a->N % 4) { me_set_error("me_gemm: K, ldx must be multiples of 8 and N, ldc of 4"); return ME_EINVAL; }
  if (((uintptr_t)a->X | (uintptr_t)a->W) & 15 || ((uintptr_t)a->C & 7)) { me_set_error("me_gemm: misaligned pointer"); return ME_EINVAL; }
  if (a->gather < 0 || a->gather > 2) { me_set_error("me_gemm: bad gather mode"); return ME_EINVAL; }
  if (a->gather == ME_GATHER_CONV3) {
    if (a->Hin <= 0 || a->Win <= 0 || a->Hout <= 0 || a->Wout <= 0 || (a->stride != 1 && a->stride != 2) || a->ups < 0 || a->ups > 2 ||
        (a->pad0 != 0 && a->pad0 != 1) || a->M % (a->Hout * a->Wout)) { me_set_error("me_gemm: bad conv geometry"); return ME_EINVAL; }
  }
  if (a->gather == ME_GATHER_TCONV) {
    const int ftot = a->frames_total > 0 ? a->frames_total : a->frames;
    if (a->frames <= 0 || a->npix <= 0 || a->chunk <= 0 || ftot % a->chunk || (a->m_off == 0 && a->sel_rows <= a->M && a->M % (a->frames * a->npix)) || a->frame0 < 0 ||
        a->frame0 + a->frames > ftot) { me_set_error("me_gemm: bad tconv geometry"); return ME_EINVAL; }
  }
  if (a->rowvec && (a->rows_per_vec <= 0 || a->ldrv % 4 || ((uintptr_t)a->rowvec & 7))) { me_set_error("me_gemm: bad rowvec"); return ME_EINVAL; }
  if (a->res && (a->ldr % 4 || ((uintptr_t)a->res & 7))) { me_set_error("me_gemm: bad residual"); return ME_EINVAL; }
  if (a->res2 && (a->ldr2 % 4 || ((uintptr_t)a->res2 & 7))) { me_set_error("me_gemm: bad second residual"); return ME_EINVAL; }
  if (a->res_rows < 0 || a->res2_rows < 0) { me_set_error("me_gemm: negative res_rows"); return ME_EINVAL; }
  if (a->act < 0 || a->act > 2) { me_set_error("me_gemm: bad activation"); return ME_EINVAL; }
  if (a->bias && ((uintptr_t)a->bias & 7)) { me_set_error("me_gemm: misaligned bias"); return ME_EINVAL; }
  if (a->geglu && (a->N % 32 || a->rowvec || a->res || a->res2 || a->act || a->alpha != 1.0f)) { me_set_error("me_gemm: geglu needs N % 32 == 0, alpha == 1 and no rowvec/res/act"); return ME_EINVAL; }
  if (a->m_off < 0 || a->m_off >= a->M || (a->m_off > 0 && a->gather == ME_GATHER_CONV3)) { me_set_error("me_gemm: m_off must lie in [0, M) and is for dense / TemporalConv launches"); return ME_EINVAL; }
  if (a->C2 && (a->geglu || a->act || a->rowvec || a->res || a->res2 || a->c2_dh <= 0 || a->c2_dh % 8 || a->c2_col0 < 0 || a->c2_col0 % 16 || a->c2_col0 >= a->N ||
                (a->N - a->c2_col0) % a->c2_dh || a->c2_hs % 8 || a->c2_hs < (int64_t)a->M * a->c2_dh || ((uintptr_t)a->C2 & 15) || a->gather == ME_GATHER_CONV3)) {
    me_set_error("me_gemm: head-major output (C2) needs a term-free epilogue, c2_dh % 8 == 0, c2_col0 % 16 == 0, whole heads, c2_hs % 8 == 0 and >= M * c2_dh, 16-byte alignment");
    return ME_EINVAL;
  }
  hipStream_t st = reinterpret_cast<hipStream_t>(stream);
  const bool wide = a->N % 128 == 0 || a->N % 64 != 0;
  if (stage_impl() == STAGE_GLDS) {
    const int Msel = a->sel_rows > a->M ? a->sel_rows : a->M;
    const long big_blocks = (long)((Msel + 255) / 256) * (a->N / 320);
    if (a->gather == ME_GATHER_CONV3 && a->stride == 1 && a->ups == 0 && !a->pad0 && a->N % 320 == 0 && a->K % 64 == 0 && a->Hin % 16 == 0 &&
        a->Win % 16 == 0 && !a->geglu && big_blocks >= halo_min_blocks() && conv_halo())
      return launch_conv_halo(a, st);
    const bool buf = a->K % 64 == 0 && buf_stage();
    const int nit8 = (a->K / 64) * (a->gather == ME_GATHER_CONV3 ? 9 : (a->gather == ME_GATHER_TCONV ? 3 : 1));
    const bool dense = a->gather == ME_GATHER_DENSE;
    if (a->geglu && dense && buf && use_8p() > 0 && nit8 >= use_8p() && a->N % 256 == 0 && (long)((Msel + 255) / 256) * (a->N / 256) >= geglu_min_tiles())
      return launch_gemm8p<256, 256, false>(a, st);
    if (a->N % 320 == 0 && big_blocks >= big_min_blocks()) {
      if (buf && use_8p() > 0 && nit8 >= use_8p()) {
        if (!a->geglu) return dense ? launch_gemm8p<256, 320, false>(a, st) : launch_gemm8p<256, 320, true>(a, st);
        if (dense && a->N % 256 == 0 && (long)((Msel + 255) / 256) * (a->N / 256) >= big_min_blocks()) return launch_gemm8p<256, 256, false>(a, st);
      }
      return buf ? launch_gemm<256, 320, STAGE_BUF>(a, st) : launch_gemm<256, 320, STAGE_GLDS>(a, st);
    }
    if (a->N % 320 == 0 && !a->geglu && buf && use_8p() > 0 && nit8 >= min_ktiles_192() && nit8 >= use_8p() && (long)((Msel + 191) / 192) * (a->N / 320) >= min_tiles_192())
      return dense ? launch_gemm8p<192, 320, false>(a, st) : launch_gemm8p<192, 320, true>(a, st);
    if (dense && a->N % 320 == 0 && !a->geglu && buf && use_8p() > 0 && nit8 >= min_ktiles_192() && nit8 >= use_8p() && (long)((Msel + 127) / 128) * (a->N / 320) >= min_tiles_128())
      return launch_gemm8p<128, 320, false>(a, st);
    const long blocks160 = (long)((Msel + 127) / 128) * ((a->N + 159) / 160);
    {
      const long blocks128 = (long)((Msel + 127) / 128) * ((a->N + 127) / 128);
      if (a->N % 64 == 0 && blocks128 < n64_below()) return buf ? launch_gemm<128, 64, STAGE_BUF>(a, st) : launch_gemm<128, 64, STAGE_GLDS>(a, st);
    }
    if (a->N % 128 == 0 && blocks160 < 512) return buf ? launch_gemm<128, 128, STAGE_BUF>(a, st) : launch_gemm<128, 128, STAGE_GLDS>(a, st);
    if (!a->geglu && a->N % 160 == 0 && tile160()) return buf ? launch_gemm<128, 160, STAGE_BUF>(a, st) : launch_gemm<128, 160, STAGE_GLDS>(a, st);
    if (wide) return buf ? launch_gemm<128, 128, STAGE_BUF>(a, st) : launch_gemm<128, 128, STAGE_GLDS>(a, st);
    return launch_gemm<128, 64, STAGE_GLDS>(a, st);
  }
  return wide ? launch_gemm<128, 128, STAGE_REG>(a, st) : launch_gemm<128, 64, STAGE_REG>(a, st);
}
```

motioneditor_amd/models/graph.py:

```python
from __future__ import annotations

import contextlib
from dataclasses import dataclass
from typing import Callable, List, Optional, Sequence

import torch

from .. import ops, plan, segments
from ..weights import Packed

HEADS = 8
ADAPTER_CHUNK = 8
HEAD_MAJOR_Q = __import__("os").environ.get("ME_HEAD_MAJOR_Q", "1") != "0"
HEAD_MAJOR_KV = __import__("os").environ.get("ME_HEAD_MAJOR_KV", "1") != "0"
SPLIT_SHARDED_TCONV = __import__("os").environ.get("ME_SPLIT_TCONV", "1") != "0"
INPLACE_SKIPS = __import__("os").environ.get("ME_INPLACE_SKIPS", "1") != "0"
LN_FOLD = __import__("os").environ.get("ME_LN_FOLD", "1") != "0"
COND_EMBED_CACHE = True


@dataclass
class Act:
    t: torch.Tensor
    B: int
    f: int
    h: int
    w: int
    cat: Optional[torch.Tensor] = None

    @property
    def N(self) -> int:
        return self.h * self.w

    @property
    def C(self) -> int:
        return self.t.shape[1]

    def like(self, t: torch.Tensor, h: Optional[int] = None, w: Optional[int] = None) -> "Act":
        return Act(t, self.B, self.f, self.h if h is None else h, self.w if w is None else w)

    def rows_of(self, b: int) -> torch.Tensor:
        n = self.f * self.N
        return self.t[b * n:(b + 1) * n]


@dataclass
class AttnCall:
    q: torch.Tensor
    k: torch.Tensor
    v: torch.Tensor
    B: int
    f: int
    N: int
    dh: int
    nk: int
    is_cross: bool
    shard: object = None
    q_items: int = 0

    def run(self, seg_item: torch.Tensor, seg_mode: torch.Tensor, mask: Optional[torch.Tensor] = None) -> torch.Tensor:
        return ops.attention(self.q, self.k, self.v, heads=HEADS, dh=self.dh, n_items=self.B * self.f, nq=self.N, nk=self.nk,
                             seg_item=seg_item, seg_mode=seg_mode, mask=mask, **({"q_items": self.q_items} if self.q_items else {}))


@dataclass
class TemporalCall:
    q: torch.Tensor
    k: torch.Tensor
    v: torch.Tensor
    B: int
    f: int
    N: int
    dh: int
    shard: object = None
    parts: int = 0

    def run(self, kv_map: Optional[Sequence[int]] = None) -> torch.Tensor:
        if self.parts > 1:
            return ops.temporal_attention(self.q, self.k, self.v, heads=HEADS, dh=self.dh, batch=self.B, frames=self.f, npix=self.N, kv_map=kv_map,
                                          kv_parts=self.parts, q_parts=self.parts)
        if self.shard is None:
            return ops.temporal_attention(self.q, self.k, self.v, heads=HEADS, dh=self.dh, batch=self.B, frames=self.f, npix=self.N, kv_map=kv_map)
        sh = self.shard
        return ops.temporal_attention(self.q, self.k, self.v, heads=HEADS, dh=self.dh, batch=self.B, frames=sh.f_total, npix=self.N, kv_map=kv_map,
                                      q_frames=sh.f_loc, q_frame0=sh.frame0, kv_parts=sh.world)


def conv3x3(P: Packed, name: str, x: Act, stride: int = 1, ups: int = 0, **epi) -> Act:
    hv, wv = x.h << ups, x.w << ups
    ho, wo = (hv - 1) // stride + 1, (wv - 1) // stride + 1
    out = ops.gemm(x.t, P.mat(name + ".weight"), M=x.B * x.f * ho * wo, bias=P.vec(name + ".bias"),
                   conv=(x.h, x.w, ho, wo, stride, ups), **epi)
    return x.like(out, ho, wo)


def resnet_block(P: Packed, p: str, x: Act, temb: torch.Tensor, temb_off: int, *, per_frame_stats: bool, eps: float = 1e-5, shard=None,
                 out: Optional[torch.Tensor] = None) -> Act:
    rpg = x.N if per_frame_stats else x.f * x.N
    cout = P.vec(p + ".conv1.bias").shape[0]
    tv = temb[:, temb_off:temb_off + cout]
    rows_per_vec = x.t.shape[0] if temb.shape[0] == 1 else x.f * x.N
    has_t1 = P.has(p + ".temp_conv1.weight") and not P.is_zero(p + ".temp_conv1.weight", p + ".temp_conv1.bias")
    has_t2 = P.has(p + ".temp_conv2.weight") and not P.is_zero(p + ".temp_conv2.weight", p + ".temp_conv2.bias")

    gn = {}
    if shard is not None and not per_frame_stats:
        gn = dict(reduce=shard.allreduce_, rows_per_group_total=shard.f_total * x.N)
    ftot = shard.f_total if shard is not None else x.f
    rows = x.B * x.f * x.N
    h = ops.groupnorm(x.t, P.vec(p + ".norm1.weight"), P.vec(p + ".norm1.bias"), rows_per_group=rpg, eps=eps, silu=True, **gn)
    if has_t1:
        hx = torch.empty((_ext_rows(x, shard), cout), dtype=P.dtype, device=x.t.device)
        h = conv3x3(P, p + ".conv1", x.like(h), out=hx).t
        h = _tconv(P, p + ".temp_conv1", hx, x, ftot, shard, rowvec=tv, rows_per_vec=rows_per_vec, res=h)
    else:
        h = conv3x3(P, p + ".conv1", x.like(h), rowvec=tv, rows_per_vec=rows_per_vec).t
    h = ops.groupnorm(h, P.vec(p + ".norm2.weight"), P.vec(p + ".norm2.bias"), rows_per_group=rpg, eps=eps, silu=True, **gn)
    if P.has(p + ".conv_shortcut.weight"):
        sc = ops.gemm(x.t, P.mat(p + ".conv_shortcut.weight"), bias=P.vec(p + ".conv_shortcut.bias"))
    else:
        sc = x.t
    if has_t2:
        hx = torch.empty((_ext_rows(x, shard), cout), dtype=P.dtype, device=x.t.device)
        h = conv3x3(P, p + ".conv2", x.like(h), out=hx).t
        h = _tconv(P, p + ".temp_conv2", hx, x, ftot, shard, res=h, res2=sc, **({} if out is None else {"out": out}))
    else:
        h = conv3x3(P, p + ".conv2", x.like(h), res=sc, **({} if out is None else {"out": out})).t
    return x.like(h)


def _fold() -> bool:
    return LN_FOLD and not getattr(ops, "recording", False) and getattr(ops, "LN_FOLD", False)


def _gemm_st(*args, **kw):
    if _fold():
        return ops.gemm(*args, ln_out=True, **kw)
    return ops.gemm(*args, **kw), None


class LN:

    def __init__(self, P: Packed, norm: str, x: torch.Tensor, stats: Optional[torch.Tensor] = None):
        self.P, self.norm, self.x, self.stats, self._rows = P, norm, x, stats, None

    def rows(self) -> torch.Tensor:
        if self._rows is None:
            self._rows = ops.layernorm(self.x, self.P.vec(self.norm + ".weight"), self.P.vec(self.norm + ".bias"))
        return self._rows

    def gemm(self, names: Sequence[str], *, geglu_bias: Optional[str] = None, **kw):
        names = list(names)
        geglu = geglu_bias is not None
        if _fold() and self._rows is None:
            if self.stats is None:
                self.stats = ops.ln_stats(self.x)
            w, cs, cv = self.P.ln_fold(self.norm, names, geglu=geglu, bias=geglu_bias)
            return ops.gemm(self.x, w, ln=(self.stats, cs, cv, 1e-5), geglu=geglu, **kw)
        if geglu:
            return ops.gemm(self.rows(), self.P.geglu_mat(names[0]), bias=self.P.geglu_vec(geglu_bias), geglu=True, **kw)
        return ops.gemm(self.rows(), self.P.fused(names) if len(names) > 1 else self.P.mat(names[0]), **kw)


def feed_forward(P: Packed, p: str, n: "LN", res: torch.Tensor, want_stats: bool = False):
    g = n.gemm([p + ".net.0.proj.weight"], geglu_bias=p + ".net.0.proj.bias")
    return (_gemm_st if want_stats else (lambda *a, **k: (ops.gemm(*a, **k), None)))(g, P.mat(p + ".net.2.weight"), bias=P.vec(p + ".net.2.bias"), res=res)


def _ln(P: Packed, p: str, x: torch.Tensor) -> torch.Tensor:
    return ops.layernorm(x, P.vec(p + ".weight"), P.vec(p + ".bias"))


def _qkv(P: Packed, p: str, n: "LN", C: int, shard, B: int = 0, N: int = 0, head_major: bool = False):
    names = [p + ".to_q.weight", p + ".to_k.weight", p + ".to_v.weight"]
    if shard is None:
        if head_major and HEAD_MAJOR_KV and not getattr(ops, "recording", False) and getattr(ops, "HEAD_MAJOR_KV", False):
            if HEAD_MAJOR_Q:
                _, qkv = n.gemm(names, head_major=(0, C // HEADS))
                return qkv[:HEADS], qkv[HEADS:2 * HEADS], qkv[2 * HEADS:]
            q, kv = n.gemm(names, head_major=(C, C // HEADS))
            return q, kv[:HEADS], kv[HEADS:]
        qkv = n.gemm(names)
        return qkv[:, :C], qkv[:, C:2 * C], qkv[:, 2 * C:]
    ext, loc = shard.kv_buffer(n.x.shape[0], 2 * C, B, N, n.x)
    n.gemm(names[1:], out=loc)
    pending = shard.start_kv(ext, B, N, ops.copy_rows)
    q = n.gemm(names[:1])
    kv = shard.finish_kv(pending)
    return q, kv[:, :C], kv[:, C:]


def _temporal_attn(P: Packed, p: str, n: "LN", C: int, B: int, f: int, N: int, dh: int, shard, editor=None, place: str = "") -> torch.Tensor:
    def go(tc):
        return editor(call=tc, is_cross=False, place_in_unet=place, num_heads=HEADS) if editor is not None else tc.run()
    if shard is not None and shard.pixel_sharded(N):
        r = shard.to_pixel_shards(n.rows(), B * f, N, ops.copy_blocks)
        qkv = ops.gemm(r, P.fused([p + ".to_q.weight", p + ".to_k.weight", p + ".to_v.weight"]))
        a = go(TemporalCall(qkv[:, :C], qkv[:, C:2 * C], qkv[:, 2 * C:], B, shard.f_total, N // shard.world, dh, None, shard.world))
        return shard.to_frame_shards(a, B * f, N, ops.copy_blocks)
    q, k, v = _qkv(P, p, n, C, shard)
    return go(TemporalCall(q, k, v, B, f, N, dh, shard))


def _tconv(P: Packed, name: str, h_ext: torch.Tensor, x: "Act", chunk: int, shard, **epi) -> torch.Tensor:
    rows = x.B * x.f * x.N
    if shard is None:
        return ops.gemm(h_ext, P.mat(name + ".weight"), M=rows, bias=P.vec(name + ".bias"), tconv=(x.f, x.N, chunk), **epi)
    if SPLIT_SHARDED_TCONV and x.f >= 3 and getattr(ops, "ROW_RANGE", False) and not ops.gemm_splits_k(rows, P.mat(name + ".weight").shape[0], h_ext.shape[1], 3):
        w, b = P.mat(name + ".weight"), P.vec(name + ".bias")
        out = epi.pop("out", None)
        if out is None:
            out = torch.empty((rows, w.shape[0]), dtype=h_ext.dtype, device=h_ext.device)
        handle = shard.exchange_halos(h_ext, x.B, x.N, ops.copy_rows, defer=True)
        interior = (x.f, x.N, chunk, shard.frame0, shard.f_total, -1, -1)
        for bi in range(x.B):
            ops.gemm(h_ext, w, M=rows, bias=b, tconv=interior, out=out, row_range=((bi * x.f + 1) * x.N, (bi * x.f + x.f - 1) * x.N), **epi)
        hp, hn = shard.finish_halos(handle)
        full = (x.f, x.N, chunk, shard.frame0, shard.f_total, hp, hn)
        bounds = [(0, x.N)] + [((bi * x.f - 1) * x.N, (bi * x.f + 1) * x.N) for bi in range(1, x.B)] + [(rows - x.N, rows)]
        for lo, hi in bounds:
            ops.gemm(h_ext, w, M=rows, bias=b, tconv=full, out=out, row_range=(lo, hi), **epi)
        return out
    hp, hn = shard.exchange_halos(h_ext, x.B, x.N, ops.copy_rows)
    return ops.gemm(h_ext, P.mat(name + ".weight"), M=rows, bias=P.vec(name + ".bias"),
                    tconv=(x.f, x.N, chunk, shard.frame0, shard.f_total, hp, hn), **epi)


def _ext_rows(x: "Act", shard) -> int:
    return x.B * x.f * x.N + (2 * x.B * x.N if shard is not None else 0)


def basic_block(P: Packed, p: str, x: Act, text: Optional[torch.Tensor], text_seg, *, spatial, temporal, place: str,
                sc_attn: bool, has_temp: bool, shard=None, text_kv: Optional[torch.Tensor] = None, expand: int = 1, stats: Optional[torch.Tensor] = None) -> Act:
    t, C = x.t, x.C
    dh = C // HEADS
    sh1 = shard.prev_frame_view() if (shard is not None and sc_attn) else None
    q, k, v = _qkv(P, p + ".attn1", LN(P, p + ".norm1", t, stats), C, sh1, x.B, x.N, head_major=True)
    call = AttnCall(q, k, v, x.B, x.f, x.N, dh, x.N, False, sh1)
    if spatial is not None:
        a = spatial(call=call, is_cross=False, place_in_unet=place, num_heads=HEADS)
    elif sc_attn:
        a = call.run(*segments.prev_cur(x.B, x.f, t.device, sh1))
    else:
        a = call.run(*segments.self_items(x.B * x.f, t.device))
    t, st = _gemm_st(a, P.mat(p + ".attn1.to_out.0.weight"), bias=P.vec(p + ".attn1.to_out.0.bias"), res=t)
    if expand > 1 and text is None:
        raise ValueError("basic_block: expand needs the text cross-attention (that is where the batch entries start to differ)")
    if text is not None:
        q = LN(P, p + ".norm2", t, st).gemm([p + ".attn2.to_q.weight"])
        kv = text_kv if text_kv is not None else ops.gemm(text, P.fused([p + ".attn2.to_k.weight", p + ".attn2.to_v.weight"]))
        call = AttnCall(q, kv[:, :C], kv[:, C:], x.B * expand, x.f, x.N, dh, 77, True, None, x.B * x.f if expand > 1 else 0)
        if spatial is not None:
            a = spatial(call=call, is_cross=True, place_in_unet=place, num_heads=HEADS, text_seg=text_seg)
        else:
            a = call.run(*text_seg)
        if expand > 1:
            ops.SELECT_ROWS_SCALE = 1
        t, st = _gemm_st(a, P.mat(p + ".attn2.to_out.0.weight"), bias=P.vec(p + ".attn2.to_out.0.bias"), res=t, **({"res_rows": t.shape[0]} if expand > 1 else {}))
        if expand > 1:
            x = Act(t, x.B * expand, x.f, x.h, x.w)
    t, st = feed_forward(P, p + ".ff", LN(P, p + ".norm3", t, st), t, want_stats=has_temp)
    if has_temp:
        a = _temporal_attn(P, p + ".attn_temp", LN(P, p + ".norm_temp", t, st), C, x.B, x.f, x.N, dh, shard, temporal, place)
        t = ops.gemm(a, P.mat(p + ".attn_temp.to_out.0.weight"), bias=P.vec(p + ".attn_temp.to_out.0.bias"), res=t)
    return x.like(t)


def transformer2d(P: Packed, p: str, x: Act, text, text_seg, *, spatial=None, temporal=None, place: str = "", sc_attn: bool = True,
                  has_temp: bool = True, shard=None, out: Optional[torch.Tensor] = None, text_kv: Optional[dict] = None, expand: int = 1) -> Act:
    n = ops.groupnorm(x.t, P.vec(p + ".norm.weight"), P.vec(p + ".norm.bias"), rows_per_group=x.N, eps=1e-6, silu=False)
    t, st = _gemm_st(n, P.mat(p + ".proj_in.weight"), bias=P.vec(p + ".proj_in.bias"))
    t = basic_block(P, p + ".transformer_blocks.0", x.like(t), text, text_seg, spatial=spatial, temporal=temporal, place=place,
                    sc_attn=sc_attn, has_temp=has_temp, shard=shard, text_kv=None if text_kv is None else text_kv[p], expand=expand, stats=st).t
    y = ops.gemm(t, P.mat(p + ".proj_out.weight"), bias=P.vec(p + ".proj_out.bias"), res=x.t, **({} if out is None else {"out": out}),
                 **({"res_rows": x.t.shape[0]} if expand > 1 else {}))
    return Act(y, x.B * expand, x.f, x.h, x.w)


def resnet_names(n_up: bool) -> List[str]:
    names = [f"down_blocks.{i}.resnets.{j}" for i in range(4) for j in range(2)] + ["mid_block.resnets.0", "mid_block.resnets.1"]
    if n_up:
        names += [f"up_blocks.{i}.resnets.{j}" for i in range(4) for j in range(3)]
    return names


def time_embedding(P: Packed, t: float, names: List[str], device):
    e = ops.timestep_embed(1, 320, t, device)
    e = ops.gemm(e, P.mat("time_embedding.linear_1.weight"), bias=P.vec("time_embedding.linear_1.bias"), act=2)
    e = ops.gemm(e, P.mat("time_embedding.linear_2.weight"), bias=P.vec("time_embedding.linear_2.bias"), act=2)
    w = P.fused([n + ".time_emb_proj.weight" for n in names])
    b = P.fused_vec([n + ".time_emb_proj.bias" for n in names])
    temb = ops.gemm(e, w, bias=b)
    offs, o = {}, 0
    for n in names:
        offs[n] = o
        o += P.vec(n + ".conv1.bias").shape[0]
    return temb, offs


def attention_block_names(n_up: bool) -> List[str]:
    names = [f"down_blocks.{i}.attentions.{j}" for i in range(3) for j in range(2)] + ["mid_block.attentions.0"]
    if n_up:
        names += [f"up_blocks.{i}.attentions.{j}" for i in range(1, 4) for j in range(3)]
    return names


def text_kv_all(P: Packed, text: torch.Tensor, names: List[str]) -> dict:
    ws = []
    for n in names:
        t = n + ".transformer_blocks.0.attn2."
        ws += [t + "to_k.weight", t + "to_v.weight"]
    kv = ops.gemm(text, P.fused(ws))
    out, o = {}, 0
    for n in names:
        c2 = 2 * P.vec(n + ".norm.weight").shape[0]
        out[n] = kv[:, o:o + c2]
        o += c2
    return out


def adapter_block(P: Packed, p: str, x: Act, src, nb: Optional[int] = None, shard=None) -> torch.Tensor:
    t, C, dev = x.t, x.C, x.t.device
    dh = C // HEADS
    nb = x.B if nb is None else nb
    share = nb != x.B
    if share:
        assert x.B == 1
    rows_x = t.shape[0]
    if shard is None:
        tx = t
    else:
        tx = torch.empty((_ext_rows(x, shard), C), dtype=P.dtype, device=dev)
        ops.copy_rows(tx[:t.shape[0]], t)
    hc = _tconv(P, p + ".block1", tx, x, ADAPTER_CHUNK, shard, act=1)
    hc = ops.gemm(hc, P.mat(p + ".block2.weight"), bias=P.vec(p + ".block2.bias"), res=t)
    sh2 = shard.chunk_view(ADAPTER_CHUNK) if (shard is not None and shard.adapter == "halo") else shard
    q_, k_, v_ = _qkv(P, p + ".attn_temp", LN(P, p + ".norm_temp", t), C, sh2, x.B, x.N)
    a = AttnCall(q_, k_, v_, x.B, x.f, x.N, dh, x.N, False, sh2).run(*segments.first_prev_chunked(x.B, x.f, ADAPTER_CHUNK, dev, sh2))
    a = ops.gemm(a, P.mat(p + ".attn_temp.to_out.0.weight"), bias=P.vec(p + ".attn_temp.to_out.0.bias"), res=t)
    a = _ln(P, p + ".cross_pose_norm", a)
    q = ops.gemm(a, P.mat(p + ".attn_pose.to_q.weight"))
    wkv = P.fused([p + ".attn_pose.to_k.weight", p + ".attn_pose.to_v.weight"])
    if isinstance(src, (list, tuple)):
        n1 = src[0].shape[0]
        kv = torch.empty((len(src) * n1, 2 * C), dtype=P.dtype, device=dev)
        for k, part in enumerate(src):
            ops.gemm(part, wkv, out=kv[k * n1:(k + 1) * n1])
    else:
        kv = ops.gemm(src, wkv)
    seg = segments.self_items(nb * x.f, dev)
    ap = ops.attention(q, kv[:, :C], kv[:, C:], heads=HEADS, dh=dh, n_items=nb * x.f, nq=x.N, nk=x.N, seg_item=seg[0], seg_mode=seg[1],
                       **({"q_items": x.B * x.f} if share else {}))
    a, st = _gemm_st(ap, P.mat(p + ".attn_pose.to_out.0.weight"), bias=P.vec(p + ".attn_pose.to_out.0.bias"), res=a, **({"res_rows": rows_x} if share else {}))
    a, st = feed_forward(P, p + ".ff", LN(P, p + ".ff_norm", a, st), a, want_stats=True)
    at = _temporal_attn(P, p + ".attn_self_temp", LN(P, p + ".norm_self_temp", a, st), C, nb, x.f, x.N, dh, shard)
    return ops.gemm(at, P.mat(p + ".attn_self_temp.to_out.0.weight"), bias=P.vec(p + ".attn_self_temp.to_out.0.bias"), res=a, res2=hc,
                    **({"res2_rows": rows_x} if share else {}))


def adapter_pack(P: Packed, prefix: str = "controlnet_adapter.") -> List[str]:
    for i in range(12):
        p = f"{prefix}body.{i}"
        P.mat(p + ".block1.weight"), P.vec(p + ".block1.bias"), P.mat(p + ".block2.weight"), P.vec(p + ".block2.bias")
        for a in ("attn_temp", "attn_self_temp"):
            P.fused([f"{p}.{a}.to_q.weight", f"{p}.{a}.to_k.weight", f"{p}.{a}.to_v.weight"])
        P.mat(p + ".attn_pose.to_q.weight")
        P.fused([p + ".attn_pose.to_k.weight", p + ".attn_pose.to_v.weight"])
        for a in ("attn_temp", "attn_pose", "attn_self_temp"):
            P.mat(f"{p}.{a}.to_out.0.weight"), P.vec(f"{p}.{a}.to_out.0.bias")
        for n in ("norm_temp", "cross_pose_norm", "ff_norm", "norm_self_temp"):
            P.vec(f"{p}.{n}.weight"), P.vec(f"{p}.{n}.bias")
        P.geglu_mat(p + ".ff.net.0.proj.weight"), P.geglu_vec(p + ".ff.net.0.proj.bias"), P.mat(p + ".ff.net.2.weight"), P.vec(p + ".ff.net.2.bias")
    return sorted(P.trainable_ids(prefix).values())


def unet_tune_pack(P: Packed, names: Sequence[str]) -> List[str]:
    blocks = {f"{b}.transformer_blocks.0": b for b in attention_block_names(True)}
    text_kv = [f"{b}.transformer_blocks.0.attn2.{w}.weight" for b in attention_block_names(True) for w in ("to_k", "to_v")]
    keys, bad = [], []
    for n in names:
        parts = n.split(".")
        head = ".".join(parts[:5]) if parts[0] == "mid_block" else ".".join(parts[:6])
        tail = n[len(head) + 1:]
        if head not in blocks:
            bad.append(n)
            continue
        if tail in ("attn1.to_q.weight", "attn1.to_k.weight", "attn1.to_v.weight", "attn_temp.to_q.weight", "attn_temp.to_k.weight", "attn_temp.to_v.weight"):
            a = tail.split(".")[0]
            P.fused([f"{head}.{a}.to_q.weight", f"{head}.{a}.to_k.weight", f"{head}.{a}.to_v.weight"])
            keys.append("fused:" + "|".join(f"{head}.{a}.to_{x}.weight" for x in "qkv"))
        elif tail == "attn2.to_q.weight" or tail.endswith(("to_out.0.weight", "ff.net.2.weight")) and tail.split(".")[0] in ("attn1", "attn2", "attn_temp", "ff"):
            P.mat(n)
            keys.append("mat:" + n)
        elif tail.endswith(("to_out.0.bias", "ff.net.2.bias")) and tail.split(".")[0] in ("attn1", "attn2", "attn_temp", "ff"):
            P.vec(n)
            keys.append("vec:" + n)
# ... 265 lines not shown
```

motioneditor_amd/ops.py:

```python
from __future__ import annotations

import ctypes as C
from typing import Optional, Sequence, Tuple

import os

import torch

from . import capi
from .capi import AttnArgs, AttnBwdArgs, ConvSmallArgs, GemmArgs, GemmDwArgs, GroupNormArgs, LayerNormArgs, TAttnArgs

F16 = torch.float16


_raw_stream = getattr(torch._C, "_cuda_getCurrentRawStream", None)
_cur_device = getattr(torch._C, "_cuda_getDevice", None)


def _stream() -> int:
    if _raw_stream is not None and _cur_device is not None:
        return _raw_stream(_cur_device())
    return torch.cuda.current_stream().cuda_stream


def _p(t: Optional[torch.Tensor]) -> Optional[int]:
    return None if t is None else t.data_ptr()


def _chk2d(t: torch.Tensor, name: str) -> None:
    if t.dtype != F16 or t.dim() != 2 or t.stride(1) != 1 or not t.is_cuda:
        raise ValueError(f"{name}: expected a CUDA fp16 2-D tensor with unit column stride, got {t.dtype} {tuple(t.shape)} {t.stride()}")


SELECT_ROWS_SCALE = 1
PROFILE = None


def _pb():
    if PROFILE is None:
        return None
    e = torch.cuda.Event(enable_timing=True)
    e.record()
    return e


def _pe(e0, family: str, flops: float, nbytes: float, detail: str = "", kernel: str = "", exec_flops=None) -> None:
    if e0 is None:
        return
    e1 = torch.cuda.Event(enable_timing=True)
    e1.record()
    PROFILE.append((family, flops, nbytes, e0, e1, detail, kernel or family, flops if exec_flops is None else exec_flops))


def _last_kernel() -> str:
    return capi.lib().me_last_kernel().decode()


def empty(rows: int, cols: int, like: torch.Tensor) -> torch.Tensor:
    return torch.empty((rows, cols), dtype=F16, device=like.device)


ATTN_ITEM_ORDER = os.environ.get("ME_ATTN_ITEM_ORDER", "1") != "0"
ROW_RANGE = True
LN_FOLD = True
HEAD_MAJOR_KV = True


def gemm(x: torch.Tensor, w: torch.Tensor, *, M: Optional[int] = None, out: Optional[torch.Tensor] = None,
         bias: Optional[torch.Tensor] = None, rowvec: Optional[torch.Tensor] = None, rows_per_vec: int = 0,
         res: Optional[torch.Tensor] = None, res2: Optional[torch.Tensor] = None, geglu: bool = False, act: int = 0, alpha: float = 1.0,
         conv: Optional[Tuple[int, int, int, int, int, int]] = None,
         tconv: Optional[Tuple[int, ...]] = None, res_rows: int = 0, res2_rows: int = 0, head_major: Optional[Tuple[int, int]] = None,
         row_range: Optional[Tuple[int, int]] = None, ln: Optional[Tuple[torch.Tensor, torch.Tensor, torch.Tensor, float]] = None, ln_out: bool = False):
    _chk2d(x, "gemm.x")
    if w.dtype != F16 or not w.is_contiguous() or w.dim() != 3:
        raise ValueError("gemm.w: expected contiguous fp16 [N, taps, K]")
    N, taps, K = w.shape
    a = GemmArgs()
    a.gather = capi.GATHER_DENSE
    if conv is not None:
        a.gather = capi.GATHER_CONV3
        a.Hin, a.Win, a.Hout, a.Wout, a.stride, a.ups = conv[:6]
        a.pad0 = conv[6] if len(conv) > 6 else 0
        if taps != 9:
            raise ValueError("gemm: conv needs 9 taps")
    elif tconv is not None:
        a.gather = capi.GATHER_TCONV
        a.frames, a.npix, a.chunk = tconv[:3]
        if len(tconv) > 3:
            a.frame0, a.frames_total, a.halo_prev, a.halo_next = tconv[3:]
        if taps != 3:
            raise ValueError("gemm: tconv needs 3 taps")
    elif taps != 1:
        raise ValueError("gemm: dense needs 1 tap")
    if M is None:
        M = x.shape[0]
    if x.shape[1] < K:
        raise ValueError(f"gemm: x has {x.shape[1]} columns < K={K}")
    n_out = N // 2 if geglu else N
    panels = None
    if head_major is not None:
        col0, hdh = head_major
        if out is not None or geglu or (N - col0) % hdh or col0 < 0:
            raise ValueError("gemm: head_major needs whole heads behind col0 >= 0 and allocates its own outputs")
        panels = torch.empty(((N - col0) // hdh, M, hdh), dtype=F16, device=x.device)
        a.C2, a.c2_col0, a.c2_dh, a.c2_hs = panels.data_ptr(), col0, hdh, M * hdh
        n_out = col0
        if col0 == 0:
            out = panels.view(-1)[:8 * M].view(M, 8)
    if out is None:
        if row_range is not None:
            raise ValueError("gemm: row_range writes into a caller-provided `out` of all M rows")
        out = empty(M, n_out, x)
    _chk2d(out, "gemm.out")
    if out.shape[0] < M or out.shape[1] < n_out:
        raise ValueError("gemm: out too small")
    a.X, a.W, a.C = x.data_ptr(), w.data_ptr(), out.data_ptr()
    a.M, a.N, a.K = M, N, K
    if row_range is not None:
        lo, hi = row_range
        if not (0 <= lo < hi <= M) or conv is not None:
            raise ValueError("gemm: row_range must lie inside [0, M) (dense / TemporalConv launches)")
        a.m_off, a.M = lo, hi
        a.sel_rows = max(a.sel_rows, M)
    a.ldx, a.ldc = x.stride(0), out.stride(0)
    a.bias = _p(bias)
    if rowvec is not None:
        _chk2d(rowvec, "gemm.rowvec")
        a.rowvec, a.ldrv, a.rows_per_vec = rowvec.data_ptr(), rowvec.stride(0), rows_per_vec
    if res is not None:
        _chk2d(res, "gemm.res")
        a.res, a.ldr = res.data_ptr(), res.stride(0)
    if res2 is not None:
        _chk2d(res2, "gemm.res2")
        a.res2, a.ldr2 = res2.data_ptr(), res2.stride(0)
    a.geglu = 1 if geglu else 0
    a.act = act
    a.alpha = alpha
    a.res_rows, a.res2_rows = res_rows, res2_rows
    if ln is not None:
        st_, cs_, cv_, eps_ = ln
        if st_.dtype != torch.float32 or st_.dim() != 3 or st_.shape[2] != 2 or st_.stride(2) != 1 or st_.stride(1) != 2 or st_.shape[1] < M \
                or cs_.dtype != torch.float32 or cv_.dtype != torch.float32 or cs_.numel() != N or cv_.numel() != N or not cs_.is_contiguous() or not cv_.is_contiguous():
            raise ValueError("gemm: ln = (fp32 stats [parts, rows, 2], fp32 colsum [N], fp32 cvec [N], eps)")
        a.ln_stats, a.ln_colsum, a.ln_cvec, a.ln_eps = st_.data_ptr(), cs_.data_ptr(), cv_.data_ptr(), eps_
        a.ln_parts, a.ln_stride = st_.shape[0], st_.stride(0)
    so = None
    if ln_out:
        if panels is not None or geglu:
            raise ValueError("gemm: ln_out is for plain row outputs")
        so = torch.empty((n_out // 320 if n_out % 320 == 0 else 1, M, 2), dtype=torch.float32, device=x.device)
        a.ln_out, a.ln_out_stride = so.data_ptr(), so.stride(0)
    if SELECT_ROWS_SCALE > 1:
        a.sel_rows = M * SELECT_ROWS_SCALE
    for r_, n_ in ((res, res_rows), (res2, res2_rows)):
        if r_ is not None and r_.shape[0] < (n_ or M):
            raise ValueError("gemm: residual has fewer rows than the output reads")
    if N >= 1280 and M <= 8192:
        nb = capi.lib().me_gemm_work_bytes(C.byref(a))
        if nb > 0:
            a.work, a.work_bytes = _work(nb, x.device, "splitk").data_ptr(), nb
    e0 = _pb()
    capi.check(capi.lib().me_gemm(C.byref(a), _stream()), "me_gemm")
    if e0 is not None:
        rows_in = (M // (conv[2] * conv[3])) * conv[0] * conv[1] if conv is not None else M
        n_terms = (res is not None) + (res2 is not None)
        n_hm = panels.numel() // M if panels is not None else 0
        _pe(e0, "gemm", 2.0 * M * N * K * taps, 2.0 * (rows_in * K + N * K * taps + M * n_out * (1 + n_terms) + M * n_hm), f"M{M} N{N} K{K} taps{taps}{' geglu' if geglu else ''}{' +b' if bias is not None else ''}{' +rv' if rowvec is not None else ''}"
            f"{' +res' if res is not None else ''}{' +res2' if res2 is not None else ''}{' act' + str(act) if act else ''}{' a' + str(alpha) if alpha != 1.0 else ''}{' ln' if ln is not None else ''}{' lnout' if ln_out else ''}", _last_kernel())
    if panels is not None and n_out == 0:
        return None, panels
    out = out[:M, :n_out] if (out.shape[0] != M or out.shape[1] != n_out) else out
    if so is not None:
        return out, so
    return out if panels is None else (out, panels)


def ln_stats(x: torch.Tensor) -> torch.Tensor:
    _chk2d(x, "ln_stats.x")
    rows, Cc = x.shape
    st = torch.empty((Cc // 320 if Cc % 320 == 0 else 1, rows, 2), dtype=torch.float32, device=x.device)
    e0 = _pb()
    capi.check(capi.lib().me_ln_stats(x.data_ptr(), x.stride(0), rows, Cc, st.data_ptr(), st.stride(0), _stream()), "me_ln_stats")
    _pe(e0, "layernorm", 3.0 * rows * Cc, 2.0 * rows * Cc, "stats", "ln_stats")
    return st


def gemm_splits_k(M: int, N: int, K: int, taps: int = 1) -> bool:
    if not (N >= 1280 and M <= 8192):
        return False
    a = GemmArgs()
    a.M, a.N, a.K = M, N, K
    a.gather = capi.GATHER_TCONV if taps == 3 else (capi.GATHER_CONV3 if taps == 9 else capi.GATHER_DENSE)
    return capi.lib().me_gemm_work_bytes(C.byref(a)) > 0


def conv_small(inp: torch.Tensor, w: torch.Tensor, bias: Optional[torch.Tensor], *, n_img: int, Cin: int, H: int, Wd: int,
               img_stride: int, ch_stride: int, frames: int = 0, frame_stride: int = 0, silu: bool = False) -> torch.Tensor:
    if w.dtype != torch.float32 or (bias is not None and bias.dtype != torch.float32):
        raise ValueError("conv_small: weights and bias must be fp32")
    Cout = w.shape[0]
    out = torch.empty((n_img * H * Wd, Cout), dtype=F16, device=inp.device)
    a = ConvSmallArgs()
    a.inp, a.W, a.bias, a.out = inp.data_ptr(), w.data_ptr(), _p(bias), out.data_ptr()
    a.n_img, a.Cin, a.Cout, a.H, a.Wd = n_img, Cin, Cout, H, Wd
    a.img_stride, a.ch_stride = img_stride, ch_stride
    if inp.dtype == torch.float32:
        a.in_is_f16 = 0
    elif inp.dtype == F16:
        a.in_is_f16 = 1
    else:
        raise ValueError("conv_small: input must be fp32 or fp16")
    a.silu = 1 if silu else 0
    a.frames, a.frame_stride = frames, frame_stride
    capi.check(capi.lib().me_conv_small(C.byref(a), _stream()), "me_conv_small")
    return out


def attention(q: torch.Tensor, k: torch.Tensor, v: torch.Tensor, *, heads: int, dh: int, n_items: int, nq: int, nk: int,
              seg_item: torch.Tensor, seg_mode: torch.Tensor, mask: Optional[torch.Tensor] = None,
              scale: Optional[float] = None, out: Optional[torch.Tensor] = None, q_items: int = 0, lse: Optional[torch.Tensor] = None) -> torch.Tensor:
    hm = k.dim() == 3
    if hm:
        if v.dim() != 3 or k.shape[0] != heads or v.shape[0] != heads or k.shape[2] != dh or v.shape[2] != dh or k.stride(2) != 1 or v.stride(2) != 1 \
                or k.dtype != F16 or v.dtype != F16:
            raise ValueError("attention: head-major k / v must be fp16 [heads, rows, dh] with unit column stride")
        if q.dim() == 3:
            if q.shape[0] != heads or q.shape[2] != dh or q.stride(2) != 1 or q.dtype != F16 or q.stride(1) % 8 or q.stride(0) % 8 or q.data_ptr() % 16:
                raise ValueError("attention: head-major q must be fp16 [heads, rows, dh] with unit column stride")
        else:
            _chk2d(q, "attention.q")
    else:
        for t, n in ((q, "q"), (k, "k"), (v, "v")):
            _chk2d(t, "attention." + n)
    qhm = q.dim() == 3
    if q.shape[1 if qhm else 0] < (q_items or n_items) * nq:
        raise ValueError("attention: q has fewer rows than the items read")
    if seg_item.dtype != torch.int32 or seg_mode.dtype != torch.int32 or seg_item.shape != seg_mode.shape or seg_item.shape[0] != n_items:
        raise ValueError("attention: seg tables must be int32 [n_items, nseg]")
    if out is None:
        out = empty(n_items * nq, heads * dh, q)
    a = AttnArgs()
    a.Q, a.K, a.V, a.O = q.data_ptr(), k.data_ptr(), v.data_ptr(), out.data_ptr()
    a.ldq, a.ldk, a.ldv, a.ldo = q.stride(1 if qhm else 0), k.stride(1 if hm else 0), v.stride(1 if hm else 0), out.stride(0)
    if hm:
        a.hsk, a.hsv = k.stride(0), v.stride(0)
    if qhm:
        a.hsq = q.stride(0)
    a.heads, a.dh = heads, dh
    a.n_items, a.nq, a.nk, a.nseg = n_items, nq, nk, seg_item.shape[1]
    a.seg_item, a.seg_mode, a.mask = seg_item.data_ptr(), seg_mode.data_ptr(), _p(mask)
    a.scale = dh ** -0.5 if scale is None else scale
    from . import segments
    gd = segments.GENERAL_DUAL.get(seg_mode.data_ptr())
    bd = segments.BINARY_DUAL.get(seg_mode.data_ptr())
    if gd is None or bd is None:
        gd = bool(((seg_mode == 1) | (seg_mode == 2)).any().item())
        bd = bool((seg_mode == 3).any().item())
    a.general_dual = 1 if gd else 0
    a.q_items = q_items
    order = segments.ITEM_ORDER.get(seg_item.data_ptr())
    if order is not None and order.device == q.device and order.numel() == n_items and ATTN_ITEM_ORDER:
        a.item_order = order.data_ptr()
    if lse is not None:
        if lse.dtype != torch.float32 or not lse.is_contiguous() or lse.numel() != n_items * nq * heads:
            raise ValueError("attention: lse must be a contiguous fp32 [n_items * nq, heads] tensor")
        a.lse = lse.data_ptr()
    if bd and not gd:
        n_kv = k.shape[1 if hm else 0] // nk
        vsum = torch.empty(capi.lib().me_attn_vsum_bytes(n_kv, heads * dh) // 4, dtype=torch.float32, device=q.device)
        a.vsum, a.n_kv_items = vsum.data_ptr(), n_kv
    e0 = _pb()
    capi.check(capi.lib().me_attn(C.byref(a), _stream()), "me_attn")
    if e0 is not None:
        units = segments.KEY_UNITS.get(seg_item.data_ptr())
        if units is None:
            sm, si = seg_mode.tolist(), seg_item.tolist()
            units = sum((2 if m != 0 else 1) for ri, rm in zip(si, sm) for i_, m in zip(ri, rm) if i_ >= 0)
        keys = nk * units
        nseg_exec = segments.SEG_COUNT.get(seg_item.data_ptr())
        if nseg_exec is None:
            nseg_exec = int((seg_item >= 0).sum().item())
        _pe(e0, f"attn_dh{dh}", 4.0 * heads * nq * keys * dh, 2.0 * 4 * n_items * nq * heads * dh, "", _last_kernel(),
            4.0 * heads * nq * nk * nseg_exec * dh)
    return out


def temporal_attention(q: torch.Tensor, k: torch.Tensor, v: torch.Tensor, *, heads: int, dh: int, batch: int, frames: int, npix: int,
                       kv_map: Optional[Sequence[int]] = None, scale: Optional[float] = None, q_frames: int = 0, q_frame0: int = 0,
                       kv_parts: int = 1, q_parts: int = 1) -> torch.Tensor:
    for t, n in ((q, "q"), (k, "k"), (v, "v")):
        _chk2d(t, "temporal_attention." + n)
    out = empty(batch * (q_frames or frames) * npix, heads * dh, q)
    a = TAttnArgs()
    a.Q, a.K, a.V, a.O = q.data_ptr(), k.data_ptr(), v.data_ptr(), out.data_ptr()
    a.ldq, a.ldk, a.ldv, a.ldo = q.stride(0), k.stride(0), v.stride(0), out.stride(0)
    a.heads, a.dh, a.batch, a.frames, a.npix = heads, dh, batch, frames, npix
    km = list(kv_map) if kv_map is not None else list(range(batch))
    for i in range(8):
        a.kv_map[i] = km[i] if i < len(km) else 0
    a.scale = dh ** -0.5 if scale is None else scale
    a.q_frames, a.q_frame0, a.kv_parts, a.q_parts = q_frames, q_frame0, kv_parts, q_parts
    e0 = _pb()
    capi.check(capi.lib().me_tattn(C.byref(a), _stream()), "me_tattn")
    _pe(e0, "tattn", 4.0 * batch * npix * heads * frames * frames * dh, 2.0 * 4 * batch * frames * npix * heads * dh)
    return out


_gn_scratch = {}


def groupnorm(x: torch.Tensor, gamma: torch.Tensor, beta: torch.Tensor, *, rows_per_group: int, eps: float, silu: bool,
              groups: int = 32, out: Optional[torch.Tensor] = None, reduce=None, rows_per_group_total: Optional[int] = None) -> torch.Tensor:
    _chk2d(x, "groupnorm.x")
    rows, Cc = x.shape
    if out is None:
        out = empty(rows, Cc, x)
    nsg = rows // rows_per_group
    nbytes = capi.lib().me_groupnorm_scratch_bytes(rows, rows_per_group, groups)
    key = (x.device, nbytes, _stream(), torch.cuda.is_current_stream_capturing())
    stats = _gn_scratch.get(key)
    if stats is None:
        stats = _gn_scratch[key] = torch.empty(nbytes // 8, dtype=torch.float64, device=x.device)
    a = GroupNormArgs()
    a.X, a.Y, a.gamma, a.beta, a.stats = x.data_ptr(), out.data_ptr(), gamma.data_ptr(), beta.data_ptr(), stats.data_ptr()
    a.rows, a.rows_per_group, a.C, a.ldx, a.ldy = rows, rows_per_group, Cc, x.stride(0), out.stride(0)
    a.groups, a.eps, a.silu = groups, eps, 1 if silu else 0
    e0 = _pb()
    if reduce is None:
        capi.check(capi.lib().me_groupnorm(C.byref(a), _stream()), "me_groupnorm")
    else:
        capi.check(capi.lib().me_groupnorm_stats(C.byref(a), _stream()), "me_groupnorm_stats")
        reduce(stats[:nsg * groups * 2])
        capi.check(capi.lib().me_groupnorm_apply(C.byref(a), rows_per_group_total or rows_per_group, _stream()), "me_groupnorm_apply")
    _pe(e0, "groupnorm", 8.0 * rows * Cc, 4.0 * rows * Cc)
    return out


def layernorm(x: torch.Tensor, gamma: torch.Tensor, beta: torch.Tensor, eps: float = 1e-5) -> torch.Tensor:
    _chk2d(x, "layernorm.x")
    out = empty(x.shape[0], x.shape[1], x)
    a = LayerNormArgs()
    a.X, a.Y, a.gamma, a.beta = x.data_ptr(), out.data_ptr(), gamma.data_ptr(), beta.data_ptr()
    a.rows, a.C, a.ldx, a.ldy, a.eps = x.shape[0], x.shape[1], x.stride(0), out.stride(0), eps
    e0 = _pb()
    capi.check(capi.lib().me_layernorm(C.byref(a), _stream()), "me_layernorm")
    _pe(e0, "layernorm", 8.0 * x.shape[0] * x.shape[1], 4.0 * x.shape[0] * x.shape[1])
    return out


def softmax_rows(x: torch.Tensor, out: Optional[torch.Tensor] = None) -> torch.Tensor:
    if x.dtype != F16 or x.dim() != 2 or x.stride(1) != 1:
        raise ValueError("softmax_rows: expected an fp16 [rows, cols] view with unit column stride")
    if out is None:
        out = torch.empty_like(x)
    e0 = _pb()
    capi.check(capi.lib().me_softmax_rows(out.data_ptr(), out.stride(0), x.data_ptr(), x.stride(0), x.shape[0], x.shape[1], _stream()), "me_softmax_rows")
    _pe(e0, "softmax", 0.0, 4.0 * x.shape[0] * x.shape[1])
    return out


def axpy_rows(y: torch.Tensor, x: torch.Tensor, a_: torch.Tensor, alpha: float = 1.0) -> torch.Tensor:
    for t, n in ((y, "y"), (x, "x"), (a_, "a")):
        _chk2d(t, "axpy_rows." + n)
    capi.check(capi.lib().me_axpy_rows(y.data_ptr(), y.stride(0), x.data_ptr(), x.stride(0), a_.data_ptr(), a_.stride(0),
                                       y.shape[0], y.shape[1], alpha, _stream()), "me_axpy_rows")
    return y


def copy_rows(y: torch.Tensor, x: torch.Tensor) -> torch.Tensor:
    _chk2d(y, "copy_rows.y")
    _chk2d(x, "copy_rows.x")
    capi.check(capi.lib().me_copy_rows(y.data_ptr(), y.stride(0), x.data_ptr(), x.stride(0), x.shape[0], x.shape[1], _stream()), "me_copy_rows")
    return y


def copy_blocks(y: torch.Tensor, x: torch.Tensor, n0: int, n1: int, rows: int, *, ys0: int, ys1: int, xs0: int, xs1: int) -> torch.Tensor:
    _chk2d(y, "copy_blocks.y")
    _chk2d(x, "copy_blocks.x")
    if (n0 - 1) * xs0 + (n1 - 1) * xs1 + rows > x.shape[0] or (n0 - 1) * ys0 + (n1 - 1) * ys1 + rows > y.shape[0] or x.shape[1] > y.shape[1]:
        raise ValueError("copy_blocks: block grid exceeds a tensor")
    capi.check(capi.lib().me_copy_blocks(y.data_ptr(), y.stride(0), x.data_ptr(), x.stride(0), n0, n1, rows, x.shape[1], ys0, ys1, xs0, xs1, _stream()),
               "me_copy_blocks")
    return y


NATIVE = True


def clone_rows(x: torch.Tensor) -> torch.Tensor:
    return copy_rows(torch.empty_like(x), x)


def _as_f16_row(t: torch.Tensor) -> torch.Tensor:
    v = t.reshape(-1).view(F16)
    if v.numel() % 8 or v.data_ptr() % 16:
        raise ValueError("byte copy: size must be a multiple of 16 bytes and the address 16-byte aligned")
    return v.reshape(1, -1)


def repeat_batch(x: torch.Tensor, times: int) -> torch.Tensor:
    if not x.is_contiguous():
        raise ValueError("repeat_batch: contiguous input")
    out = torch.empty((times * x.shape[0],) + tuple(x.shape[1:]), dtype=x.dtype, device=x.device)
    for k in range(times):
        copy_rows(_as_f16_row(out[k * x.shape[0]:(k + 1) * x.shape[0]]), _as_f16_row(x))
    return out


def to_f16_rows(ehs: torch.Tensor) -> torch.Tensor:
    Cc = ehs.shape[-1]
    if ehs.dtype == F16 and ehs.is_contiguous():
        return ehs.reshape(-1, Cc)
    B = ehs.shape[0]
    n = ehs[0].numel() // Cc
    out = torch.empty((B * n, Cc), dtype=F16, device=ehs.device)
    parts = [(out, ehs)] if ehs.is_contiguous() else [(out[b * n:(b + 1) * n], ehs[b]) for b in range(B)]
    for dst, src in parts:
        if not src.is_contiguous():
            raise ValueError("to_f16_rows: batch entries must be contiguous")
        if src.dtype == torch.float32:
            cast_f16(dst, src)
        elif src.dtype == F16:
            copy_rows(dst, src.reshape(-1, Cc))
        else:
            raise ValueError(f"to_f16_rows: unsupported dtype {src.dtype}")
    return out


def silu(x: torch.Tensor) -> torch.Tensor:
    out = torch.empty_like(x)
    capi.check(capi.lib().me_silu(out.data_ptr(), x.data_ptr(), x.numel(), _stream()), "me_silu")
    return out


def relu(x: torch.Tensor) -> torch.Tensor:
    out = torch.empty_like(x)
    capi.check(capi.lib().me_relu(out.data_ptr(), x.data_ptr(), x.numel(), _stream()), "me_relu")
    return out


def quick_gelu(x: torch.Tensor) -> torch.Tensor:
    if x.dtype != F16 or not x.is_contiguous():
        raise ValueError("quick_gelu: contiguous fp16 input")
    out = torch.empty_like(x)
    capi.check(capi.lib().me_quick_gelu(out.data_ptr(), x.data_ptr(), x.numel(), _stream()), "me_quick_gelu")
    return out


def embed_rows(tok: torch.Tensor, pos: torch.Tensor, ids: torch.Tensor, seq: int) -> torch.Tensor:
    if tok.dtype != F16 or pos.dtype != F16 or tok.dim() != 2 or pos.dim() != 2 or not tok.is_contiguous() or not pos.is_contiguous() or tok.shape[1] != pos.shape[1]:
        raise ValueError("embed_rows: tok [vocab, C] and pos [seq, C] must be contiguous fp16 tables of one width")
    if ids.dtype != torch.int32 or not ids.is_contiguous() or ids.device != tok.device or seq <= 0 or seq > pos.shape[0] or ids.numel() % seq:
        raise ValueError("embed_rows: ids must be a contiguous int32 device tensor of n * seq entries, seq <= the position table")
    rows, Cc = ids.numel(), tok.shape[1]
    out = torch.empty((rows, Cc), dtype=F16, device=tok.device)
    capi.check(capi.lib().me_embed_rows(out.data_ptr(), tok.data_ptr(), pos.data_ptr(), ids.data_ptr(), rows, seq, Cc, tok.shape[0], _stream()), "me_embed_rows")
    return out


def attention_causal(q: torch.Tensor, k: torch.Tensor, v: torch.Tensor, *, heads: int, dh: int, n_seq: int, nq: int, scale: Optional[float] = None) -> torch.Tensor:
    for t, n in ((q, "q"), (k, "k"), (v, "v")):
        _chk2d(t, "attention_causal." + n)
        if t.shape[0] < n_seq * nq or t.shape[1] < heads * dh:
            raise ValueError(f"attention_causal.{n}: expected at least [{n_seq * nq}, {heads * dh}], got {tuple(t.shape)}")
    out = empty(n_seq * nq, heads * dh, q)
    capi.check(capi.lib().me_attn_causal(out.data_ptr(), out.stride(0), q.data_ptr(), q.stride(0), k.data_ptr(), k.stride(0), v.data_ptr(), v.stride(0),
                                         n_seq, heads, dh, nq, dh ** -0.5 if scale is None else scale, _stream()), "me_attn_causal")
    return out


def _not_in_a_plan(what: str) -> None:
# ... 434 lines not shown
```

motioneditor_amd/weights.py:

```python
from __future__ import annotations

from typing import Callable, Dict, Iterable, List, Mapping, Optional, Sequence, Tuple

import numpy as np
import torch


def _t(v) -> torch.Tensor:
    if isinstance(v, np.ndarray):
        return torch.from_numpy(v)
    return v.detach().cpu()


def select_trainable(names: Iterable[str], trainable_modules: Sequence[str] = (), trainable_params: Sequence[str] = ()) -> List[str]:
    mods, pars = tuple(trainable_modules), tuple(trainable_params)
    out = []
    for n in names:
        parts = n.split(".")
        if (mods and any(".".join(parts[:i]).endswith(mods) for i in range(1, len(parts)))) or (pars and n.endswith(pars)):
            out.append(n)
    return out


class Packed:

    def __init__(self, state: Mapping[str, object], device, prefix: str = "", dtype=torch.float16):
        self.state = state
        self.dtype = dtype
        self.device = torch.device(device)
        self.prefix = prefix
        self.cache: Dict[str, torch.Tensor] = {}
        self.live: Dict[str, Callable[[], torch.Tensor]] = {}

    def make_private(self) -> None:
        if not getattr(self, "_private", False):
            self.state = dict(self.state)
            self._private = True

    def has(self, name: str) -> bool:
        return (self.prefix + name) in self.state

    def raw(self, name: str) -> torch.Tensor:
        src = self.live.get(name)
        if src is not None:
            return src().float()
        return _t(self.state[self.prefix + name]).float()

    def _put(self, key: str, t: torch.Tensor) -> torch.Tensor:
        d = t.to(self.dtype).contiguous().to(self.device)
        self.cache[key] = d
        return d

    @staticmethod
    def _as_taps(w: torch.Tensor) -> torch.Tensor:
        if w.dim() == 2:
            return w[:, None, :]
        if w.dim() == 4:
            co, ci, kh, kw = w.shape
            return w.permute(0, 2, 3, 1).reshape(co, kh * kw, ci)
        if w.dim() == 3:
            return w.permute(0, 2, 1)
        raise ValueError(f"unsupported weight rank {w.dim()}")

    @staticmethod
    def _geglu_perm(n_out: int) -> torch.Tensor:
        q = torch.arange(n_out // 16)
        val = (q[:, None] * 16 + torch.arange(16)[None]).reshape(-1, 16)
        gate = val + n_out
        return torch.cat([val, gate], dim=1).reshape(-1)

    def packed_f32(self, key: str) -> torch.Tensor:
        kind, _, names = key.partition(":")
        ns = names.split("|")
        if kind == "vec":
            return self.raw(names).reshape(-1)
        if kind == "mat":
            return self._as_taps(self.raw(names)).contiguous()
        if kind == "fused":
            return torch.cat([self._as_taps(self.raw(n)) for n in ns], dim=0).contiguous()
        if kind == "fvec":
            return torch.cat([self.raw(n).reshape(-1) for n in ns])
        if kind == "geglu":
            w = self.raw(names)
            return w[self._geglu_perm(w.shape[0] // 2)][:, None, :].contiguous()
        if kind == "gegluv":
            b = self.raw(names)
            return b[self._geglu_perm(b.shape[0] // 2)].contiguous()
        raise KeyError(key)

    def _get(self, key: str) -> torch.Tensor:
        hit = self.cache.get(key)
        return hit if hit is not None else self._put(key, self.packed_f32(key))

    def vec(self, name: str) -> torch.Tensor:
        return self._get("vec:" + name)

    def mat(self, name: str) -> torch.Tensor:
        return self._get("mat:" + name)

    def mat32(self, name: str) -> torch.Tensor:
        k = "mat32:" + name
        if k not in self.cache:
            self.cache[k] = self._as_taps(self.raw(name)).contiguous().to(self.device)
        return self.cache[k]

    def vec32(self, name: str) -> torch.Tensor:
        k = "vec32:" + name
        if k not in self.cache:
            self.cache[k] = self.raw(name).reshape(-1).contiguous().to(self.device)
        return self.cache[k]

    def fused(self, names: Iterable[str]) -> torch.Tensor:
        return self._get("fused:" + "|".join(names))

    def fused_vec(self, names: Iterable[str]) -> torch.Tensor:
        return self._get("fvec:" + "|".join(names))

    def geglu_mat(self, name: str) -> torch.Tensor:
        return self._get("geglu:" + name)

    def geglu_vec(self, name: str) -> torch.Tensor:
        return self._get("gegluv:" + name)

    def ln_fold(self, norm: str, names: Iterable[str], geglu: bool = False, bias: Optional[str] = None):
        names = list(names)
        key = ("lnwg:" if geglu else "lnw:") + "|".join([norm + ".weight", norm + ".bias", *names, *([bias] if bias else [])])
        hit = self.cache.get(key)
        if hit is None:
            gamma, beta = self.raw(norm + ".weight").reshape(-1), self.raw(norm + ".bias").reshape(-1)
            if geglu:
                w = self.packed_f32("geglu:" + names[0])
                b = self.packed_f32("gegluv:" + bias) if bias else None
            else:
                w = torch.cat([self._as_taps(self.raw(n)) for n in names], dim=0)
                b = self.raw(bias).reshape(-1) if bias else None
            if w.shape[1] != 1:
                raise ValueError("ln_fold: dense projections only")
            wq = (w * gamma[None, None, :]).to(self.dtype).contiguous()
            colsum = wq.float().sum(dim=(1, 2))
            cvec = w[:, 0, :] @ beta
            if b is not None:
                cvec = cvec + b
            hit = (wq.to(self.device), colsum.contiguous().to(self.device), cvec.float().contiguous().to(self.device))
            self.cache[key] = hit
        return hit

    def is_zero(self, *names: str) -> bool:
        k = "zero:" + "|".join(names)
        if k not in self.cache:
            self.cache[k] = all(bool((self.raw(n) == 0).all()) for n in names)
        return bool(self.cache[k])

    def trainable_ids(self, name_prefix: str) -> Dict[int, str]:
        out = {}
        for key, t in self.cache.items():
            kind, _, names = key.partition(":")
            if isinstance(t, torch.Tensor) and kind in ("mat", "vec", "fused", "fvec", "geglu", "gegluv") and all(n.startswith(name_prefix) for n in names.split("|")):
                out[id(t)] = key
        return out

    def row_ranges(self, key: str) -> List[Tuple[int, int, str]]:
        kind, _, names = key.partition(":")
        ns = names.split("|")
        rows_of = lambda n: int(self.state[self.prefix + n].shape[0])
        if kind in ("lnw", "lnwg"):
            ns = [n for n in ns[2:] if n.endswith(".weight")]
            if kind == "lnwg":
                return [(0, rows_of(ns[0]), ns[0])]
        out, r = [], 0
        for n in ns:
            rows = rows_of(n)
            out.append((r, r + rows, n))
            r += rows
        return out

    def trainable_rows(self, keys: Iterable[str], names: Iterable[str]) -> Dict[int, List[Tuple[int, int, str]]]:
        names = set(names)
        out: Dict[int, List[Tuple[int, int, str]]] = {}
        for key in keys:
            rr = [r for r in self.row_ranges(key) if r[2] in names]
            if rr:
                out[id(self.cache[key])] = rr
        return out

    def update(self, name: str, value: torch.Tensor) -> None:
        from . import ops
        self.make_private()
        self.state[self.prefix + name] = value.detach().cpu().clone()
        stale = [k for k in self.cache if name in k.partition(":")[2].split("|")]
        if self.device.type == "cuda":
            ops.invalidate_transposed([self.cache[k] for k in stale if isinstance(self.cache[k], torch.Tensor) and self.cache[k].dim() == 3])
        for key in stale:
            del self.cache[key]

    def rehome(self, key: str, storage: torch.Tensor) -> torch.Tensor:
        t = self._get(key)
        if storage.dtype != t.dtype or storage.numel() != t.numel() or not storage.is_contiguous():
            raise ValueError("rehome: storage must be a contiguous slice of the packed tensor's dtype and size")
        storage.copy_(t.reshape(-1))
        v = storage.view(t.shape)
        self.cache[key] = v
        return v

    def unpack_grad(self, key: str, g: torch.Tensor) -> Dict[str, torch.Tensor]:
        kind, _, names = key.partition(":")
        names_l = names.split("|")
        g = g.float().cpu()

        def untap(n: str, t: torch.Tensor) -> torch.Tensor:
            shp = self.raw(n).shape
            if len(shp) == 2:
                return t[:, 0, :]
            if len(shp) == 4:
                return t.reshape(shp[0], shp[2], shp[3], shp[1]).permute(0, 3, 1, 2)
            return t.permute(0, 2, 1)

        if kind == "mat":
            return {names: untap(names, g)}
        if kind == "vec":
            return {names: g.reshape(self.raw(names).shape)}
        if kind in ("fused", "fvec"):
            out, r0 = {}, 0
            for n in names_l:
                rows = self.raw(n).shape[0]
                out[n] = untap(n, g[r0:r0 + rows]) if kind == "fused" else g[r0:r0 + rows]
                r0 += rows
            return out
        if kind in ("geglu", "gegluv"):
            n_out = g.shape[0] // 2
            inv = torch.empty(2 * n_out, dtype=torch.long)
            inv[self._geglu_perm(n_out)] = torch.arange(2 * n_out)
            return {names: (g[inv][:, 0, :] if kind == "geglu" else g[inv])}
        raise KeyError(key)

    def nbytes(self) -> int:
        return sum(t.numel() * t.element_size() for t in self.cache.values() if isinstance(t, torch.Tensor))
```

Baseline: 6.851.

## Fold nearest-upsample into 3x3 conv as four 2x2 sub-pixel convolutions

A nearest-neighbor 2x upsample followed by a 3x3 conv is rewritten as four parity-specific 2x2 convolutions over the low-resolution input. The folded 16-tap weights are precomputed on the host, and the GEMM kernels gain an UPS3 instantiation. That instantiation gathers the four taps directly from the input and scatters output rows to interleaved positions through a row map. This cuts the MACs for upsampling convs from 9 to 4 taps per output and skips gathering zero or duplicated upsampled pixels. The cost is extra template instantiations, scattered stores, split-K being disabled for this path, and weight caching that is bypassed for live or rehomed weights.

```diff
diff --git a/motioneditor_amd/csrc/gemm.hip b/motioneditor_amd/csrc/gemm.hip
--- a/motioneditor_amd/csrc/gemm.hip
+++ b/motioneditor_amd/csrc/gemm.hip
@@ -38,14 +38,22 @@
   bool valid;
 };
 
-__device__ __forceinline__ RowInfo make_row(const me_gemm_args& a, int m) {
+__device__ __forceinline__ RowInfo make_row(const me_gemm_args& a, int m, int par = 0, bool ups3 = false) {
   RowInfo r;
   r.valid = m < a.M;
   r.base = m;
   r.y0 = 0;
   r.x0 = 0;
   if (!r.valid) return r;
-  if (a.gather == ME_GATHER_CONV3) {
+  if (ups3) {
+    const int hw = a.Hin * a.Win;
+    const int img = m / hw;
+    const int rem = m - img * hw;
+    const int y = rem / a.Win;
+    r.base = img * hw;
+    r.y0 = y + (par >> 1) - 1;
+    r.x0 = rem - y * a.Win + (par & 1) - 1;
+  } else if (a.gather == ME_GATHER_CONV3) {
     const int hw = a.Hout * a.Wout;
     const int img = m / hw;
     const int rem = m - img * hw;
@@ -62,9 +70,14 @@
   return r;
 }
 
-__device__ __forceinline__ int src_row(const me_gemm_args& a, const RowInfo& r, int tap) {
+__device__ __forceinline__ int src_row(const me_gemm_args& a, const RowInfo& r, int tap, bool ups3 = false) {
   if (!r.valid) return -1;
   if (a.gather == ME_GATHER_DENSE) return r.base;
+  if (ups3) {
+    const int iy = r.y0 + (tap >> 1), ix = r.x0 + (tap & 1);
+    if (iy < 0 || iy >= a.Hin || ix < 0 || ix >= a.Win) return -1;
+    return r.base + iy * a.Win + ix;
+  }
   if (a.gather == ME_GATHER_CONV3) {
     const int ky = tap / 3, kx = tap - ky * 3;
     const int iy = r.y0 + ky, ix = r.x0 + kx;
@@ -82,6 +95,11 @@
   if (ls >= 0 && ls < a.frames) return r.base + dt * a.npix;
   const int hb = ls < 0 ? a.halo_prev : a.halo_next;
   return hb < 0 ? -1 : hb + r.x0;
+}
+
+__device__ __forceinline__ int out_row(const me_gemm_args& a, const RowInfo& r, int par) {
+  const int py = par >> 1, px = par & 1;
+  return r.base * 4 + (2 * (r.y0 + 1 - py) + py) * a.Wout + 2 * (r.x0 + 1 - px) + px;
 }
 
 template <int NT, int MT, int WN>
@@ -333,8 +351,9 @@
 }
 
 struct LnOutCtx { int m0, wr, wc, tid; char* red; };
-template <int F, int NT, int MT, int WN>
-__device__ __forceinline__ void epilogue_rowpass(const me_gemm_args& a, f32x4 (&acc)[NT][MT], int mw0, int nw0, int lane, char* scr, const LnOutCtx& lnx) {
+template <int F, int NT, int MT, int WN, bool OMAP = false>
+__device__ __forceinline__ void epilogue_rowpass(const me_gemm_args& a, f32x4 (&acc)[NT][MT], int mw0, int nw0, int lane, char* scr, const LnOutCtx& lnx, const int* otab = nullptr) {
+  static_assert(!OMAP || F == 0, "the output-row map serves the term-free epilogue");
   static_assert(F >= 0 && (F & 1) == 0 && MT % 2 == 0 && WN % 16 == 0, "row-pass epilogue");
   constexpr bool has_rv = (F & 2) != 0, has_res = (F & 4) != 0, has_res2 = (F & 8) != 0;
   constexpr int NCHK = MT / 2, ROWS = 32, CH = WN / 8, PIECES = ROWS * CH, IT = PIECES / 64, PITCH = WN * 2 + 16;
@@ -438,7 +457,11 @@
     for (int t = 0; t < IT; ++t) {
       const int m = mw0 + c * ROWS + prow[t];
       if (m >= a.M) continue;
-      f16* dst = C + (long)m * a.ldc + pcol[t];
+      long mo = m;
+      if constexpr (OMAP) {
+        if (otab) mo = otab[m - lnx.m0];
+      }
+      f16* dst = C + mo * a.ldc + pcol[t];
       if (c2 && hoff[t] >= 0) dst = reinterpret_cast<f16*>(a.C2) + (long)m * a.c2_dh + hoff[t];
       st16(dst, d[t].u);
     }
@@ -666,7 +689,7 @@
   }
 }
 
-template <int BM, int BN, int STAGE, int WM = 64>
+template <int BM, int BN, int STAGE, int WM = 64, bool UPS3 = false>
 __global__ __launch_bounds__(BM / WM * 128, WM == 128 ? 1 : 2) void gemm_kernel(const me_gemm_args a) {
   constexpr int NTHR = BM / WM * 128;
   constexpr int RSTR = NTHR / 8;
@@ -688,16 +711,19 @@
 
   const int nbn = (a.N + BN - 1) / BN;
   const int nbm = (a.M - a.m_off + BM - 1) / BM;
-  const int w = xcd_remap(blockIdx.x, nbm * nbn);
-  const int tile_n = w % nbn, tile_m = w / nbn;
+  constexpr bool ups3 = UPS3;
+  const int w = xcd_remap(blockIdx.x, nbm * nbn * (ups3 ? 4 : 1));
+  const int tile_n = w % nbn, tile_mp = w / nbn;
+  const int par = ups3 ? tile_mp / nbm : 0, tile_m = tile_mp - par * nbm;
   const int m0 = a.m_off + tile_m * BM, n0 = tile_n * BN;
 
+  const int taps = a.gather == ME_GATHER_CONV3 ? (ups3 ? 4 : 9) : (a.gather == ME_GATHER_TCONV ? 3 : 1);
+  const int wtaps = ups3 ? 16 : taps;
   const f16* __restrict__ X = reinterpret_cast<const f16*>(a.X);
-  const f16* __restrict__ W = reinterpret_cast<const f16*>(a.W);
-
-  const int taps = a.gather == ME_GATHER_CONV3 ? 9 : (a.gather == ME_GATHER_TCONV ? 3 : 1);
+  const f16* __restrict__ W = reinterpret_cast<const f16*>(a.W) + (long)(4 * par) * a.K;
+
   const int nkc = (a.K + BK - 1) / BK;
-  const bool packk = STAGE == STAGE_GLDS && a.gather == ME_GATHER_CONV3 && a.K < BK && BK % a.K == 0;
+  const bool packk = STAGE == STAGE_GLDS && a.gather == ME_GATHER_CONV3 && !ups3 && a.K < BK && BK % a.K == 0;
   const int nit = packk ? (9 * a.K + BK - 1) / BK : taps * nkc;
 
   int srow, scol;
@@ -711,7 +737,7 @@
 
   RowInfo rinfo[XROWS];
 #pragma unroll
-  for (int i = 0; i < XROWS; ++i) rinfo[i] = make_row(a, m0 + srow + RSTR * i);
+  for (int i = 0; i < XROWS; ++i) rinfo[i] = make_row(a, m0 + srow + RSTR * i, par, ups3);
 
   long xoff[XROWS];
   int cur_tap = -1;
@@ -720,7 +746,7 @@
       cur_tap = tap;
 #pragma unroll
       for (int i = 0; i < XROWS; ++i) {
-        const int s = src_row(a, rinfo[i], tap);
+        const int s = src_row(a, rinfo[i], tap, ups3);
         xoff[i] = s < 0 ? -1L : (long)s * a.ldx;
       }
     }
@@ -764,18 +790,18 @@
     typedef __attribute__((address_space(3))) void* lptr_t;
     constexpr unsigned OOB = 0x80000000u;
     long brow = m0;
-    if (a.gather == ME_GATHER_CONV3) brow = (long)(m0 / (a.Hout * a.Wout)) * a.Hin * a.Win;
+    if (a.gather == ME_GATHER_CONV3) brow = (long)(m0 / (ups3 ? a.Hin * a.Win : a.Hout * a.Wout)) * a.Hin * a.Win;
     else if (a.gather == ME_GATHER_TCONV) brow = m0 > a.npix ? m0 - a.npix : 0;
     const auto xsrd = __builtin_amdgcn_make_buffer_rsrc(const_cast<f16*>(X + brow * a.ldx), 0, OOB, 0x00020000);
     const int wrows = min(a.N - n0, BN);
-    const auto wsrd = __builtin_amdgcn_make_buffer_rsrc(const_cast<f16*>(W + (long)n0 * taps * a.K), 0, (unsigned)((long)wrows * taps * a.K * 2), 0x00020000);
+    const auto wsrd = __builtin_amdgcn_make_buffer_rsrc(const_cast<f16*>(W + (long)n0 * wtaps * a.K), 0, (unsigned)(((long)(wrows - 1) * wtaps + taps) * a.K * 2), 0x00020000);
     unsigned xo[XROWS], wo[WROWS];
 #pragma unroll
-    for (int i = 0; i < WROWS; ++i) wo[i] = (unsigned)(((long)(srow + RSTR * i) * taps * a.K + scol) * 2);
+    for (int i = 0; i < WROWS; ++i) wo[i] = (unsigned)(((long)(srow + RSTR * i) * wtaps * a.K + scol) * 2);
     auto set_tap_off = [&](int tap) {
 #pragma unroll
       for (int i = 0; i < XROWS; ++i) {
-        const int sr = src_row(a, rinfo[i], tap);
+        const int sr = src_row(a, rinfo[i], tap, ups3);
         xo[i] = sr < 0 ? OOB : (unsigned)(((long)(sr - brow) * a.ldx + scol) * 2);
       }
     };
@@ -843,7 +869,7 @@
 #pragma unroll
       for (int i = 0; i < WROWS; ++i) {
         const int n = n0 + srow + RSTR * i;
-        const f16* src = (kok && n < a.N) ? W + (long)n * taps * a.K + wk : zsrc;
+        const f16* src = (kok && n < a.N) ? W + (long)n * wtaps * a.K + wk : zsrc;
         __builtin_amdgcn_global_load_lds((gptr_t)src, (lptr_t)(dw + i * (RSTR * 128)), 16, 0, 0);
       }
     };
@@ -867,7 +893,7 @@
 #pragma unroll
       for (int i = 0; i < WROWS; ++i) {
         const int n = n0 + srow + RSTR * i;
-        rw[i] = (kok && n < a.N) ? ldg128(W + ((long)n * taps + tap) * a.K + c) : zero128();
+        rw[i] = (kok && n < a.N) ? ldg128(W + ((long)n * wtaps + tap) * a.K + c) : zero128();
       }
     };
     auto sstore = [&](int buf) {
@@ -894,10 +920,11 @@
   const int ncols = a.geglu ? BN / 2 : BN;
   const int Nout = a.geglu ? a.N / 2 : a.N;
   constexpr bool CFITS = (size_t)BM * (BN + 8) <= (size_t)2 * (BM + BN) * LD;
-  const bool wide_store = CFITS && (Nout % 8 == 0) && (a.ldc % 8 == 0) && ((reinterpret_cast<uintptr_t>(a.C) & 15) == 0) && !a.C2;
+  const bool wide_store = CFITS && (Nout % 8 == 0) && (a.ldc % 8 == 0) && ((reinterpret_cast<uintptr_t>(a.C) & 15) == 0) && !a.C2 && !ups3;
   auto rowfn = [&](int i) {
     const int m = m0 + wm * WM + i * 16 + (lane & 15);
-    return m < a.M ? m : -1;
+    if (m >= a.M) return -1;
+    return ups3 ? out_row(a, make_row(a, m, par, true), par) : m;
   };
   if (!wide_store) {
     epilogue<NT, MT, WN>(a, acc, rowfn, m0, n0, wn, lane, nullptr, 0);
@@ -1030,8 +1057,9 @@
   epilogue<NT, MT, WN>(a, acc, rowfn, 0, n0, wn, lane, nullptr, 0);
 }
 
-template <int BM, int BN, bool GATHER, int EPI>
+template <int BM, int BN, bool GATHER, int EPI, bool UPS3 = false>
 __global__ __launch_bounds__(512, 2) void gemm8p_kernel(const me_gemm_args a) {
+  static_assert(!UPS3 || (GATHER && BN == 320 && EPI <= 0), "ups 3: gather kernels, term-free row pass or direct epilogues");
   constexpr int WN = BN / 4, NT = WN / 16, NT0 = (NT + 1) / 2, NT1 = NT / 2;
   constexpr int GR = BM / 2, HALF = GR / 2, MH = HALF / 16, MT = 2 * MH;
   constexpr int NPA = 2 * HALF / 8;
@@ -1046,15 +1074,20 @@
 
   const int nbn = (a.N + BN - 1) / BN;
   const int nbm = (a.M - a.m_off + BM - 1) / BM;
-  const int w = xcd_remap(blockIdx.x, nbm * nbn);
+  constexpr bool ups3 = UPS3;
+  const int nbmp = ups3 ? 4 * nbm : nbm;
+  const int w = xcd_remap(blockIdx.x, nbmp * nbn);
   int tile_n, tile_m;
-  if (a.splits_ & TILEORDER_FLAG) { tile_m = w % nbm; tile_n = w / nbm; }
+  if (a.splits_ & TILEORDER_FLAG) { tile_m = w % nbmp; tile_n = w / nbmp; }
   else { tile_n = w % nbn; tile_m = w / nbn; }
+  const int par = ups3 ? tile_m / nbm : 0;
+  tile_m -= par * nbm;
   const int m0 = a.m_off + tile_m * BM, n0 = tile_n * BN;
 
   const f16* __restrict__ X = reinterpret_cast<const f16*>(a.X);
-  const f16* __restrict__ W = reinterpret_cast<const f16*>(a.W);
-  const int taps = !GATHER ? 1 : (a.gather == ME_GATHER_CONV3 ? 9 : (a.gather == ME_GATHER_TCONV ? 3 : 1));
+  const int taps = !GATHER ? 1 : (a.gather == ME_GATHER_CONV3 ? (ups3 ? 4 : 9) : (a.gather == ME_GATHER_TCONV ? 3 : 1));
+  const int wtaps = ups3 ? 16 : taps;
+  const f16* __restrict__ W = reinterpret_cast<const f16*>(a.W) + (long)(4 * par) * a.K;
   const int nkc = a.K / BK;
   const int nit = taps * nkc;
 
@@ -1062,12 +1095,12 @@
   constexpr unsigned OOB = 0x80000000u;
   long brow = m0;
   if (GATHER) {
-    if (a.gather == ME_GATHER_CONV3) brow = (long)(m0 / (a.Hout * a.Wout)) * a.Hin * a.Win;
+    if (a.gather == ME_GATHER_CONV3) brow = (long)(m0 / (ups3 ? a.Hin * a.Win : a.Hout * a.Wout)) * a.Hin * a.Win;
     else if (a.gather == ME_GATHER_TCONV) brow = m0 > a.npix ? m0 - a.npix : 0;
   }
   const auto xsrd = __builtin_amdgcn_make_buffer_rsrc(const_cast<f16*>(X + brow * a.ldx), 0, OOB, 0x00020000);
   const int wrows = min(a.N - n0, BN);
-  const auto wsrd = __builtin_amdgcn_make_buffer_rsrc(const_cast<f16*>(W + (long)n0 * taps * a.K), 0, (unsigned)((long)wrows * taps * a.K * 2), 0x00020000);
+  const auto wsrd = __builtin_amdgcn_make_buffer_rsrc(const_cast<f16*>(W + (long)n0 * wtaps * a.K), 0, (unsigned)(((long)(wrows - 1) * wtaps + taps) * a.K * 2), 0x00020000);
 
   const int prow = lane >> 3;
   const int scol = ((lane & 7) ^ ((4 * (wave & 1) + (lane >> 4)) & 7)) * 8;
@@ -1094,11 +1127,12 @@
   unsigned xo[2][2];
   if constexpr (GATHER) {
     const int r = tid & 255;
-    const RowInfo ri = make_row(a, r < BM ? m0 + r : a.M);
+    const RowInfo ri = make_row(a, r < BM ? m0 + r : a.M, par, ups3);
     for (int tap = tid >> 8; tap < taps; tap += 2) {
-      const int sr = src_row(a, ri, tap);
+      const int sr = src_row(a, ri, tap, ups3);
       tab[tap * 256 + r] = sr < 0 ? OOB : (unsigned)((long)(sr - brow) * a.ldx * 2);
     }
+    if (ups3 && tid < 256) tab[4 * 256 + r] = ri.valid ? (unsigned)out_row(a, ri, par) : ~0u;
     __syncthreads();
   } else {
 #pragma unroll
@@ -1111,9 +1145,9 @@
   }
   unsigned wo0[NT0], wo1[NT1];
 #pragma unroll
-  for (int i = 0; i < NT0; ++i) wo0[i] = (unsigned)(((long)(rB0[i] + prow) * taps * a.K + scol) * 2);
-#pragma unroll
-  for (int i = 0; i < NT1; ++i) wo1[i] = (unsigned)(((long)(rB1[i] + prow) * taps * a.K + scol) * 2);
+  for (int i = 0; i < NT0; ++i) wo0[i] = (unsigned)(((long)(rB0[i] + prow) * wtaps * a.K + scol) * 2);
+#pragma unroll
+  for (int i = 0; i < NT1; ++i) wo1[i] = (unsigned)(((long)(rB1[i] + prow) * wtaps * a.K + scol) * 2);
 
   struct Cur { int tap, kc, tl; };
   Cur cA0 = {0, 0, 0}, cA1 = {0, 0, 0};
@@ -1292,10 +1326,11 @@
     char* scr = smem + wave * (32 * (WN * 2 + 16));
     const int mw0 = m0 + wr * GR, nw0 = n0 + wc * WN;
     const LnOutCtx lnx = {m0, wr, wc, tid, smem + 8 * (32 * (WN * 2 + 16))};
-    return epilogue_rowpass<EPI, NT, MT, WN>(a, acc, mw0, nw0, lane, scr, lnx);
+    return epilogue_rowpass<EPI, NT, MT, WN, UPS3 && EPI == 0>(a, acc, mw0, nw0, lane, scr, lnx, ups3 ? reinterpret_cast<const int*>(tab + 4 * 256) : nullptr);
   } else {
     auto rowfn = [&](int i) {
       const int m = m0 + wr * GR + i * 16 + (lane & 15);
+      if constexpr (UPS3) return (int)tab[4 * 256 + wr * GR + i * 16 + (lane & 15)];
       return m < a.M ? m : -1;
     };
     epilogue<NT, MT, WN>(a, acc, rowfn, m0, n0, wc, lane, nullptr, 0);
@@ -1357,7 +1392,7 @@
   return e ? atol(e) : 400;
 }
 int choose_split(const me_gemm_args* a, long blocks, int nit) {
-  if (a->geglu || a->K % 64 || a->N < 1280 || blocks >= split_below() || nit < 32 || a->C2 || a->m_off || a->ln_stats) return 1;
+  if (a->geglu || a->K % 64 || a->N < 1280 || blocks >= split_below() || nit < 32 || a->C2 || a->m_off || a->ln_stats || (a->gather == ME_GATHER_CONV3 && a->ups == 3)) return 1;
   int S = (int)((640 + blocks - 1) / blocks);
   if (S > 4) S = 4;
   if (S > nit / 4) S = nit / 4;
@@ -1374,12 +1409,8 @@
 }
 
 long big_min_blocks() {
-  static long v = -1;
-  if (v < 0) {
-    const char* e = getenv("ME_GEMM_BIG_MIN");
-    v = e ? atol(e) : 512;
-  }
-  return v;
+  const char* e = getenv("ME_GEMM_BIG_MIN");
+  return e ? atol(e) : 512;
 }
 
 long halo_min_blocks() {
@@ -1472,7 +1503,7 @@
 
 static thread_local bool g_ln_fused = false;
 
-template <int BM, int BN, int STAGE, int WM = 64>
+template <int BM, int BN, int STAGE, int WM = 64, bool UPS3 = false>
 static int launch_gemm(const me_gemm_args* a, hipStream_t st) {
   const size_t lds = (size_t)2 * (BM + BN) * (STAGE != STAGE_REG ? BK : BK + 8) * sizeof(f16);
   static bool attr_set_dev[64] = {};
@@ -1480,13 +1511,15 @@
   (void)hipGetDevice(&dev_id);
   bool& attr_set = attr_set_dev[dev_id & 63];
   if (!attr_set) {
-    if (hipFuncSetAttribute(reinterpret_cast<const void*>(&gemm_kernel<BM, BN, STAGE, WM>), hipFuncAttributeMaxDynamicSharedMemorySize, (int)lds) != hipSuccess) {
+    if (hipFuncSetAttribute(reinterpret_cast<const void*>(&gemm_kernel<BM, BN, STAGE, WM, UPS3>), hipFuncAttributeMaxDynamicSharedMemorySize, (int)lds) != hipSuccess) {
       me_set_error("me_gemm: hipFuncSetAttribute(MaxDynamicSharedMemorySize) failed");
       return ME_EHIP;
     }
     attr_set = true;
   }
-  const int nbm = (a->M - a->m_off + BM - 1) / BM, nbn = (a->N + BN - 1) / BN;
+  constexpr int pm = UPS3 ? 4 : 1;
+  if (UPS3 != (a->gather == ME_GATHER_CONV3 && a->ups == 3)) { me_set_error("me_gemm: internal: ups = 3 launch on the wrong instantiation"); return ME_EINVAL; }
+  const int nbm = (a->M - a->m_off + BM - 1) / BM * pm, nbn = (a->N + BN - 1) / BN;
   (void)hipGetLastError();
   me_gemm_args b = *a;
   b.splits_ = 0;
@@ -1499,11 +1532,11 @@
   }
   if (S > 1) {
     b.splits_ = S;
-    hipLaunchKernelGGL((gemm_kernel<BM, BN, STAGE, WM>), dim3(nbm * nbn, S), dim3(BM / WM * 128), lds, st, b);
+    hipLaunchKernelGGL((gemm_kernel<BM, BN, STAGE, WM, UPS3>), dim3(nbm * nbn, S), dim3(BM / WM * 128), lds, st, b);
     const long vec = (long)a->M * (a->N / 4);
     hipLaunchKernelGGL(gemm_splitk_reduce_kernel, dim3((unsigned)((vec + 255) / 256 < 4096 ? (vec + 255) / 256 : 4096)), dim3(256), 0, st, b);
   } else {
-    hipLaunchKernelGGL((gemm_kernel<BM, BN, STAGE, WM>), dim3(nbm * nbn), dim3(BM / WM * 128), lds, st, b);
+    hipLaunchKernelGGL((gemm_kernel<BM, BN, STAGE, WM, UPS3>), dim3(nbm * nbn), dim3(BM / WM * 128), lds, st, b);
   }
   {
     char nm[64];
@@ -1517,7 +1550,7 @@
   return ME_OK;
 }
 
-template <int BM, int BN, bool GATHER, int EPI>
+template <int BM, int BN, bool GATHER, int EPI, bool UPS3 = false>
 static int launch_gemm8p_epi(const me_gemm_args& b, hipStream_t st) {
   const int lds = 2 * (BM + BN) * 128 + (GATHER ? 9 * 256 * 4 : (EPI == 0 ? LN_LDS_BYTES : 0));
   static bool attr_set_dev[64] = {};
@@ -1525,14 +1558,15 @@
   (void)hipGetDevice(&dev_id);
   bool& attr_set = attr_set_dev[dev_id & 63];
   if (!attr_set) {
-    if (hipFuncSetAttribute(reinterpret_cast<const void*>(&gemm8p_kernel<BM, BN, GATHER, EPI>), hipFuncAttributeMaxDynamicSharedMemorySize, lds) != hipSuccess) {
+    if (hipFuncSetAttribute(reinterpret_cast<const void*>(&gemm8p_kernel<BM, BN, GATHER, EPI, UPS3>), hipFuncAttributeMaxDynamicSharedMemorySize, lds) != hipSuccess) {
       me_set_error("me_gemm: hipFuncSetAttribute(MaxDynamicSharedMemorySize) failed");
       return ME_EHIP;
     }
     attr_set = true;
   }
-  const int nbm = (b.M - b.m_off + BM - 1) / BM, nbn = (b.N + BN - 1) / BN;
-  hipLaunchKernelGGL((gemm8p_kernel<BM, BN, GATHER, EPI>), dim3(nbm * nbn), dim3(512), lds, st, b);
+  constexpr int pm = UPS3 ? 4 : 1;
+  const int nbm = (b.M - b.m_off + BM - 1) / BM * pm, nbn = (b.N + BN - 1) / BN;
+  hipLaunchKernelGGL((gemm8p_kernel<BM, BN, GATHER, EPI, UPS3>), dim3(nbm * nbn), dim3(512), lds, st, b);
   return ME_OK;
 }
 
@@ -1545,7 +1579,8 @@
   {
     auto al = [](const void* p, int ld) { return p == nullptr || (ld % 8 == 0 && (reinterpret_cast<uintptr_t>(p) & 15) == 0); };
     const int f = (a->rowvec ? 2 : 0) | (a->res ? 4 : 0) | (a->res2 ? 8 : 0);
-    if (BN == 320 && row_epilogue() && !a->geglu && a->act == 0 && a->N % 320 == 0 && (f == 0 || f == 2 || f == 4 || f == 6 || f == 12) && al(a->C, a->ldc) &&
+    const bool ups3 = a->gather == ME_GATHER_CONV3 && a->ups == 3;
+    if (BN == 320 && !(ups3 && f != 0) && row_epilogue() && !a->geglu && a->act == 0 && a->N % 320 == 0 && (f == 0 || f == 2 || f == 4 || f == 6 || f == 12) && al(a->C, a->ldc) &&
         al(a->rowvec, a->ldrv) && al(a->res, a->ldr) && al(a->res2, a->ldr2) && (!a->C2 || f == 0))
       epi = f;
     if (tile_order_exp()) b.splits_ |= TILEORDER_FLAG;
@@ -1555,7 +1590,11 @@
     if (!g_ln_fused) b.ln_out = nullptr;
   }
   int rc;
-  if constexpr (BN == 256) {
+  const bool ups3_launch = a->gather == ME_GATHER_CONV3 && a->ups == 3;
+  if (ups3_launch) {
+    if constexpr (GATHER && BN == 320) rc = epi == 0 ? launch_gemm8p_epi<BM, BN, true, 0, true>(b, st) : launch_gemm8p_epi<BM, BN, true, -1, true>(b, st);
+    else { me_set_error("me_gemm: internal: ups = 3 launch on a kernel without the mode"); return ME_EINVAL; }
+  } else if constexpr (BN == 256) {
     rc = epi == 0 ? launch_gemm8p_epi<BM, BN, GATHER, 0>(b, st) : launch_gemm8p_epi<BM, BN, GATHER, -1>(b, st);
   } else {
     switch (epi) {
@@ -1645,8 +1684,12 @@
   if (((uintptr_t)a->X | (uintptr_t)a->W) & 15 || ((uintptr_t)a->C & 7)) { me_set_error("me_gemm: misaligned pointer"); return ME_EINVAL; }
   if (a->gather < 0 || a->gather > 2) { me_set_error("me_gemm: bad gather mode"); return ME_EINVAL; }
   if (a->gather == ME_GATHER_CONV3) {
-    if (a->Hin <= 0 || a->Win <= 0 || a->Hout <= 0 || a->Wout <= 0 || (a->stride != 1 && a->stride != 2) || a->ups < 0 || a->ups > 2 ||
+    if (a->Hin <= 0 || a->Win <= 0 || a->Hout <= 0 || a->Wout <= 0 || (a->stride != 1 && a->stride != 2) || a->ups < 0 || a->ups > 3 ||
         (a->pad0 != 0 && a->pad0 != 1) || a->M % (a->Hout * a->Wout)) { me_set_error("me_gemm: bad conv geometry"); return ME_EINVAL; }
+    if (a->ups == 3 && (a->stride != 1 || a->pad0 || a->Hout != 2 * a->Hin || a->Wout != 2 * a->Win || a->geglu)) {
+      me_set_error("me_gemm: ups = 3 (folded nearest 2x) needs stride 1, pad0 = 0, Hout = 2 Hin, Wout = 2 Win and weights [N, 16, K]");
+      return ME_EINVAL;
+    }
   }
   if (a->gather == ME_GATHER_TCONV) {
     const int ftot = a->frames_total > 0 ? a->frames_total : a->frames;
@@ -1667,15 +1710,25 @@
     return ME_EINVAL;
   }
   hipStream_t st = reinterpret_cast<hipStream_t>(stream);
+  me_gemm_args par_args;
+  const int pm = a->gather == ME_GATHER_CONV3 && a->ups == 3 ? 4 : 1;
+  if (pm == 4) {
+    par_args = *a;
+    par_args.M = a->M / 4;
+    par_args.sel_rows = a->sel_rows / 4;
+    par_args.ln_out = nullptr;
+    a = &par_args;
+  }
+#define ME_LAUNCH_GEMM(BM_, BN_, STAGE_) (pm == 4 ? launch_gemm<BM_, BN_, STAGE_, 64, true>(a, st) : launch_gemm<BM_, BN_, STAGE_>(a, st))
   const bool wide = a->N % 128 == 0 || a->N % 64 != 0;
-  if (stage_impl() == STAGE_GLDS) {
+  if (stage_impl() == STAGE_GLDS || pm == 4) {
     const int Msel = a->sel_rows > a->M ? a->sel_rows : a->M;
-    const long big_blocks = (long)((Msel + 255) / 256) * (a->N / 320);
+    const long big_blocks = (long)((Msel + 255) / 256) * pm * (a->N / 320);
     if (a->gather == ME_GATHER_CONV3 && a->stride == 1 && a->ups == 0 && !a->pad0 && a->N % 320 == 0 && a->K % 64 == 0 && a->Hin % 16 == 0 &&
         a->Win % 16 == 0 && !a->geglu && big_blocks >= halo_min_blocks() && conv_halo())
       return launch_conv_halo(a, st);
     const bool buf = a->K % 64 == 0 && buf_stage();
-    const int nit8 = (a->K / 64) * (a->gather == ME_GATHER_CONV3 ? 9 : (a->gather == ME_GATHER_TCONV ? 3 : 1));
+    const int nit8 = (a->K / 64) * (a->gather == ME_GATHER_CONV3 ? (pm == 4 ? 4 : 9) : (a->gather == ME_GATHER_TCONV ? 3 : 1));
     const bool dense = a->gather == ME_GATHER_DENSE;
     if (a->geglu && dense && buf && use_8p() > 0 && nit8 >= use_8p() && a->N % 256 == 0 && (long)((Msel + 255) / 256) * (a->N / 256) >= geglu_min_tiles())
       return launch_gemm8p<256, 256, false>(a, st);
@@ -1684,21 +1737,22 @@
         if (!a->geglu) return dense ? launch_gemm8p<256, 320, false>(a, st) : launch_gemm8p<256, 320, true>(a, st);
         if (dense && a->N % 256 == 0 && (long)((Msel + 255) / 256) * (a->N / 256) >= big_min_blocks()) return launch_gemm8p<256, 256, false>(a, st);
       }
-      return buf ? launch_gemm<256, 320, STAGE_BUF>(a, st) : launch_gemm<256, 320, STAGE_GLDS>(a, st);
-    }
-    if (a->N % 320 == 0 && !a->geglu && buf && use_8p() > 0 && nit8 >= min_ktiles_192() && nit8 >= use_8p() && (long)((Msel + 191) / 192) * (a->N / 320) >= min_tiles_192())
+      return buf ? ME_LAUNCH_GEMM(256, 320, STAGE_BUF) : ME_LAUNCH_GEMM(256, 320, STAGE_GLDS);
+    }
+    if (a->N % 320 == 0 && !a->geglu && buf && use_8p() > 0 && nit8 >= min_ktiles_192() && nit8 >= use_8p() && (long)((Msel + 191) / 192) * pm * (a->N / 320) >= min_tiles_192())
       return dense ? launch_gemm8p<192, 320, false>(a, st) : launch_gemm8p<192, 320, true>(a, st);
     if (dense && a->N % 320 == 0 && !a->geglu && buf && use_8p() > 0 && nit8 >= min_ktiles_192() && nit8 >= use_8p() && (long)((Msel + 127) / 128) * (a->N / 320) >= min_tiles_128())
       return launch_gemm8p<128, 320, false>(a, st);
-    const long blocks160 = (long)((Msel + 127) / 128) * ((a->N + 159) / 160);
+    const long blocks160 = (long)((Msel + 127) / 128) * pm * ((a->N + 159) / 160);
     {
-      const long blocks128 = (long)((Msel + 127) / 128) * ((a->N + 127) / 128);
-      if (a->N % 64 == 0 && blocks128 < n64_below()) return buf ? launch_gemm<128, 64, STAGE_BUF>(a, st) : launch_gemm<128, 64, STAGE_GLDS>(a, st);
-    }
-    if (a->N % 128 == 0 && blocks160 < 512) return buf ? launch_gemm<128, 128, STAGE_BUF>(a, st) : launch_gemm<128, 128, STAGE_GLDS>(a, st);
-    if (!a->geglu && a->N % 160 == 0 && tile160()) return buf ? launch_gemm<128, 160, STAGE_BUF>(a, st) : launch_gemm<128, 160, STAGE_GLDS>(a, st);
-    if (wide) return buf ? launch_gemm<128, 128, STAGE_BUF>(a, st) : launch_gemm<128, 128, STAGE_GLDS>(a, st);
-    return launch_gemm<128, 64, STAGE_GLDS>(a, st);
-  }
+      const long blocks128 = (long)((Msel + 127) / 128) * pm * ((a->N + 127) / 128);
+      if (a->N % 64 == 0 && blocks128 < n64_below()) return buf ? ME_LAUNCH_GEMM(128, 64, STAGE_BUF) : ME_LAUNCH_GEMM(128, 64, STAGE_GLDS);
+    }
+    if (a->N % 128 == 0 && blocks160 < 512) return buf ? ME_LAUNCH_GEMM(128, 128, STAGE_BUF) : ME_LAUNCH_GEMM(128, 128, STAGE_GLDS);
+    if (!a->geglu && a->N % 160 == 0 && tile160()) return buf ? ME_LAUNCH_GEMM(128, 160, STAGE_BUF) : ME_LAUNCH_GEMM(128, 160, STAGE_GLDS);
+    if (wide) return buf ? ME_LAUNCH_GEMM(128, 128, STAGE_BUF) : ME_LAUNCH_GEMM(128, 128, STAGE_GLDS);
+    return ME_LAUNCH_GEMM(128, 64, STAGE_GLDS);
+  }
+#undef ME_LAUNCH_GEMM
   return wide ? launch_gemm<128, 128, STAGE_REG>(a, st) : launch_gemm<128, 64, STAGE_REG>(a, st);
 }
diff --git a/motioneditor_amd/models/graph.py b/motioneditor_amd/models/graph.py
--- a/motioneditor_amd/models/graph.py
+++ b/motioneditor_amd/models/graph.py
@@ -89,9 +89,19 @@
 def conv3x3(P: Packed, name: str, x: Act, stride: int = 1, ups: int = 0, **epi) -> Act:
     hv, wv = x.h << ups, x.w << ups
     ho, wo = (hv - 1) // stride + 1, (wv - 1) // stride + 1
-    out = ops.gemm(x.t, P.mat(name + ".weight"), M=x.B * x.f * ho * wo, bias=P.vec(name + ".bias"),
-                   conv=(x.h, x.w, ho, wo, stride, ups), **epi)
+    w = None
+    if ups == 1 and stride == 1 and ups_fold_on():
+        w = P.mat_ups(name + ".weight")
+    if w is not None:
+        ups = 3
+    else:
+        w = P.mat(name + ".weight")
+    out = ops.gemm(x.t, w, M=x.B * x.f * ho * wo, bias=P.vec(name + ".bias"), conv=(x.h, x.w, ho, wo, stride, ups), **epi)
     return x.like(out, ho, wo)
+
+
+def ups_fold_on() -> bool:
+    return not getattr(ops, "recording", False) and getattr(ops, "UPS_FOLD", False) and __import__("os").environ.get("ME_UPS_FOLD", "1") != "0"
 
 
 def resnet_block(P: Packed, p: str, x: Act, temb: torch.Tensor, temb_off: int, *, per_frame_stats: bool, eps: float = 1e-5, shard=None,
diff --git a/motioneditor_amd/ops.py b/motioneditor_amd/ops.py
--- a/motioneditor_amd/ops.py
+++ b/motioneditor_amd/ops.py
@@ -63,6 +63,7 @@
 ATTN_ITEM_ORDER = os.environ.get("ME_ATTN_ITEM_ORDER", "1") != "0"
 ROW_RANGE = True
 LN_FOLD = True
+UPS_FOLD = True
 HEAD_MAJOR_KV = True
 
 
@@ -82,8 +83,8 @@
         a.gather = capi.GATHER_CONV3
         a.Hin, a.Win, a.Hout, a.Wout, a.stride, a.ups = conv[:6]
         a.pad0 = conv[6] if len(conv) > 6 else 0
-        if taps != 9:
-            raise ValueError("gemm: conv needs 9 taps")
+        if taps != (16 if a.ups == 3 else 9):
+            raise ValueError("gemm: conv needs 9 taps (16 folded ones at ups = 3)")
     elif tconv is not None:
         a.gather = capi.GATHER_TCONV
         a.frames, a.npix, a.chunk = tconv[:3]
@@ -166,8 +167,11 @@
         rows_in = (M // (conv[2] * conv[3])) * conv[0] * conv[1] if conv is not None else M
         n_terms = (res is not None) + (res2 is not None)
         n_hm = panels.numel() // M if panels is not None else 0
-        _pe(e0, "gemm", 2.0 * M * N * K * taps, 2.0 * (rows_in * K + N * K * taps + M * n_out * (1 + n_terms) + M * n_hm), f"M{M} N{N} K{K} taps{taps}{' geglu' if geglu else ''}{' +b' if bias is not None else ''}{' +rv' if rowvec is not None else ''}"
-            f"{' +res' if res is not None else ''}{' +res2' if res2 is not None else ''}{' act' + str(act) if act else ''}{' a' + str(alpha) if alpha != 1.0 else ''}{' ln' if ln is not None else ''}{' lnout' if ln_out else ''}", _last_kernel())
+        ref_taps, exec_flops = taps, None
+        if taps == 16:
+            ref_taps, exec_flops = 9, 2.0 * M * N * K * 4
+        _pe(e0, "gemm", 2.0 * M * N * K * ref_taps, 2.0 * (rows_in * K + N * K * ref_taps + M * n_out * (1 + n_terms) + M * n_hm), f"M{M} N{N} K{K} taps{taps}{' geglu' if geglu else ''}{' +b' if bias is not None else ''}{' +rv' if rowvec is not None else ''}"
+            f"{' +res' if res is not None else ''}{' +res2' if res2 is not None else ''}{' act' + str(act) if act else ''}{' a' + str(alpha) if alpha != 1.0 else ''}{' ln' if ln is not None else ''}{' lnout' if ln_out else ''}", _last_kernel(), exec_flops)
     if panels is not None and n_out == 0:
         return None, panels
     out = out[:M, :n_out] if (out.shape[0] != M or out.shape[1] != n_out) else out
diff --git a/motioneditor_amd/weights.py b/motioneditor_amd/weights.py
--- a/motioneditor_amd/weights.py
+++ b/motioneditor_amd/weights.py
@@ -31,6 +31,7 @@
         self.prefix = prefix
         self.cache: Dict[str, torch.Tensor] = {}
         self.live: Dict[str, Callable[[], torch.Tensor]] = {}
+        self._rehomed: set = set()
 
     def make_private(self) -> None:
         if not getattr(self, "_private", False):
@@ -97,6 +98,25 @@
 
     def mat(self, name: str) -> torch.Tensor:
         return self._get("mat:" + name)
+
+    @staticmethod
+    def fold_ups(w: torch.Tensor) -> torch.Tensor:
+        n, cin = w.shape[:2]
+        out = torch.zeros((n, 2, 2, 2, 2, cin), dtype=w.dtype)
+        for py in range(2):
+            for px in range(2):
+                for ky in range(3):
+                    for kx in range(3):
+                        out[:, py, px, (py + ky + 1) // 2 - py, (px + kx + 1) // 2 - px] += w[:, :, ky, kx]
+        return out.reshape(n, 16, cin)
+
+    def mat_ups(self, name: str) -> Optional[torch.Tensor]:
+        if name in self.live or ("mat:" + name) in self._rehomed:
+            self.cache.pop("ups4:" + name, None)
+            return None
+        key = "ups4:" + name
+        hit = self.cache.get(key)
+        return hit if hit is not None else self._put(key, self.fold_ups(self.raw(name)))
 
     def mat32(self, name: str) -> torch.Tensor:
         k = "mat32:" + name
@@ -200,6 +220,7 @@
         storage.copy_(t.reshape(-1))
         v = storage.view(t.shape)
         self.cache[key] = v
+        self._rehomed.add(key)
         return v
 
     def unpack_grad(self, key: str, g: torch.Tensor) -> Dict[str, torch.Tensor]:
```

Result: faster. 6.962, median of 6 (+1.6%).
